# huggingface/distil-whisper

Hardware: AMD Instinct MI355X
Metric: training audio-seconds/s (distil-large-v3 student, 30 s clips) (higher is better)
Workload: dtype bf16

## Files before the change

### distil_whisper_amd/build.py

```python
import os
import subprocess
import sys

HERE = os.path.dirname(os.path.abspath(__file__))
CSRC = os.path.join(HERE, "csrc")
LIB = os.path.join(HERE, "libdwamd.so")
SOURCES = ["gemm.hip", "gemm_tile256.hip", "gemm_tile128.hip", "gemm_wp8_nn.hip", "gemm_wp8_nt.hip", "gemm_wp8_m320.hip", "gemm_wp8_m128.hip",
           "gemm_wp16_nn.hip", "gemm_wp16_tt.hip", "gemm_wp16_small.hip", "gemm_skinny.hip", "attention.hip", "norm.hip", "loss.hip", "logmel.hip", "elementwise.hip", "optim.hip", "decode.hip", "beam.hip", "align.hip", "score.hip", "dropout.hip", "assist.hip"]
FLAGS = ["--offload-arch=gfx950", "-O3", "-std=c++17", "-fPIC", "-ffp-contract=fast", "-munsafe-fp-atomics"]


def kernels_sha16() -> str:
    import hashlib
    h = hashlib.sha256()
    files = sorted(os.path.join(CSRC, f) for f in os.listdir(CSRC) if f.endswith((".hip", ".h")))
    files.append(os.path.join(HERE, "..", "include", "dwamd.h"))
    for f in files:
        h.update(os.path.basename(f).encode())
        with open(f, "rb") as fh:
            h.update(fh.read())
    return h.hexdigest()[:16]


def _stale(obj, deps):
    if not os.path.exists(obj):
        return True
    t = os.path.getmtime(obj)
    return any(os.path.getmtime(d) > t for d in deps)


def build(force: bool = False, verbose: bool = False) -> str:
    hipcc = os.environ.get("HIPCC", "/opt/rocm/bin/hipcc")
    objdir = os.path.join(HERE, "build")
    os.makedirs(objdir, exist_ok=True)
    headers = [os.path.join(CSRC, "common.h"), os.path.join(CSRC, "gemm_common.h"), os.path.join(CSRC, "gemm_kernel.h"), os.path.join(CSRC, "gemm_wp.h"), os.path.join(CSRC, "gemm_wp16.h"), os.path.join(CSRC, "select_rules.h"),
               os.path.join(HERE, "..", "include", "dwamd.h")]
    objs, procs = [], []
    flags = FLAGS + (["-DDW_ABLATE"] if os.environ.get("DW_ABLATE") else [])
    flags += os.environ.get("DW_EXTRA_FLAGS", "").split()
    for src in SOURCES:
        s = os.path.join(CSRC, src)
        o = os.path.join(objdir, src.replace(".hip", ".o"))
        objs.append(o)
        if force or _stale(o, [s] + headers):
            cmd = [hipcc] + flags + ["-c", s, "-o", o]
            if verbose:
                print(" ".join(cmd))
            procs.append((src, subprocess.Popen(cmd, stdout=subprocess.PIPE, stderr=subprocess.STDOUT)))
    for src, p in procs:
        out, _ = p.communicate()
        if p.returncode != 0:
            sys.stderr.write(out.decode())
            raise RuntimeError(f"hipcc failed on {src}")
    if force or procs or _stale(LIB, objs):
        cmd = [hipcc, "--offload-arch=gfx950", "-shared", "-fPIC", "-o", LIB] + objs
        subprocess.check_call(cmd)
    return LIB



if __name__ == "__main__":
    print(build(force="--force" in sys.argv, verbose=True))
```

### distil_whisper_amd/csrc/attention.hip

```cpp
#include "common.h"
#include "../../include/dwamd.h"

#define NEG_BIG (-1.0e30f)
#ifndef DW_ATTN_DEFER
#define DW_ATTN_DEFER 8
#endif
#ifndef DW_ATTN_IDLE_SKIP
#define DW_ATTN_IDLE_SKIP 1
#endif
typedef __attribute__((ext_vector_type(4))) unsigned u32x4;

struct AttnP {
    const bf16* q; const bf16* k; const bf16* v; bf16* o; float* lse;
    const bf16* d_o; float* delta; bf16* dq; bf16* dk; bf16* dv;
    long ldq, ldk, ldv, ldo, lddo, lddq, lddk, lddv;
    int B, H, Lq, Lk;
    long q_rows, kv_rows;
    float* dq_colsum;
    float* dv_colsum;
    const int* q_start; const int* q_len;
    const int* kv_start; const int* kv_len;
    int kv_B;
    int plain_order;
    float defer;
    int coff;
    float scale;
};

__device__ __forceinline__ bf16x8 pack8(const f32x16& x, int s2) {
    bf16x8 r;
#pragma unroll
    for (int e = 0; e < 8; ++e) r[e] = f2bf(x[s2 * 8 + e]);
    return r;
}

__device__ __forceinline__ bf16x8 ldg8(const bf16* base, long row, long ld, int col) {
    return *(const bf16x8*)(base + row * ld + col);
}

__device__ __forceinline__ void store_t(bf16* base, long ld, long row, bool ok, int cb, int hi, const f32x16& a,
                                        float mul) {
    if (!ok) return;
#pragma unroll
    for (int g = 0; g < 4; ++g) {
        bf16x4 w;
#pragma unroll
        for (int e = 0; e < 4; ++e) w[e] = f2bf(a[g * 4 + e] * mul);
#ifdef DW_NT_ATTN
        __builtin_nontemporal_store(w, (bf16x4*)(base + row * ld + cb * 32 + g * 8 + hi * 4));
#else
        *(bf16x4*)(base + row * ld + cb * 32 + g * 8 + hi * 4) = w;
#endif
    }
}

#ifndef DW_ATTN_ROWSTORE
#define DW_ATTN_ROWSTORE 1
#endif
__device__ __forceinline__ void store_rows(bf16* base, long ld, int row0, int nrows, char* patch, int lane,
                                           const f32x16& a0, const f32x16& a1, float mul) {
    const int hi = lane >> 5, ln = lane & 31;
    char* const wr = patch + ln * 144 + hi * 8;
#pragma unroll
    for (int cb = 0; cb < 2; ++cb) {
        const f32x16& a = cb == 0 ? a0 : a1;
#pragma unroll
        for (int g = 0; g < 4; ++g) {
            bf16x4 w;
#pragma unroll
            for (int e = 0; e < 4; ++e) w[e] = f2bf(a[g * 4 + e] * mul);
            *(bf16x4*)(wr + cb * 64 + g * 16) = w;
        }
    }
    const int rr = lane >> 3, sc = lane & 7;
    u32x4 o[4];
#pragma unroll
    for (int it = 0; it < 4; ++it) o[it] = *(const u32x4*)(patch + (it * 8 + rr) * 144 + sc * 16);
    const unsigned loff = (unsigned)(rr * (int)ld + sc * 8) * 2u;
    char* const rb = (char*)(base + (long)row0 * ld);
#pragma unroll
    for (int it = 0; it < 4; ++it)
        if (row0 + it * 8 + rr < nrows) *(u32x4*)(rb + (long)it * 8 * ld * 2 + loff) = o[it];
}

__device__ __forceinline__ void colsum_t(float* colsum, bool ok, int cb, int hi, int ln, const f32x16& a, float mul) {
#pragma unroll
    for (int r = 0; r < 16; ++r) {
        float v = ok ? bf2f(f2bf(a[r] * mul)) : 0.f;
#pragma unroll
        for (int o = 1; o < 32; o <<= 1) v += __shfl_xor(v, o);
        if (ln == 0) atomicAdd(colsum + cb * 32 + (r & 3) + 8 * (r >> 2) + 4 * hi, v);
    }
}

__device__ __forceinline__ void attn_workgroup(int ntile, int H, bool plain, int& tile, int& h, int& b) {
    const int n = gridDim.x, L = blockIdx.x;
    const int xcd = L & 7, slot = L >> 3, q = n >> 3, r = n & 7;
    const int logical = plain ? L : xcd * q + min(xcd, r) + slot;
    tile = logical % ntile;
    const int bh = logical / ntile;
    h = bh % H;
    b = bh / H;
}

template <bool CAUSAL, int NW = 4, int ABL = 0, bool VL = false>
__global__ __launch_bounds__(64 * NW, CAUSAL ? 2 : 4) void attn_fwd_kernel(const AttnP p) {
    __shared__ __attribute__((aligned(1024))) char smem[2 * 16384];
    const int lane = threadIdx.x & 63;
    const int wave = __builtin_amdgcn_readfirstlane(threadIdx.x >> 6);
    const int hi = lane >> 5, ln = lane & 31;
    int tile, h, b;
    attn_workgroup((p.Lq + 32 * NW - 1) / (32 * NW), p.H, p.plain_order, tile, h, b);
    const int qb0 = tile * (32 * NW);
    long q_row0 = (long)b * p.q_rows, kv_row0 = (long)b * p.kv_rows;
    int Lq = p.Lq, Lk = p.Lk;
    if constexpr (VL) {
        q_row0 = p.q_start[b];
        Lq = p.q_len[b];
        if (p.kv_start) { kv_row0 = p.kv_start[b]; Lk = p.kv_len[b]; }
        else kv_row0 = (long)min(b, p.kv_B - 1) * p.kv_rows;
        if (qb0 >= Lq) return;
    }
    const int q = qb0 + wave * 32 + ln;
    const bool q_ok = q < Lq;
    const int qc = q_ok ? q : Lq - 1;
    const bf16* Q = p.q + q_row0 * p.ldq + h * 64;
    const bf16* K = p.k + kv_row0 * p.ldk + h * 64;
    const bf16* V = p.v + kv_row0 * p.ldv + h * 64;

    bf16x8 qf[4];
#pragma unroll
    for (int kk = 0; kk < 4; ++kk) qf[kk] = ldg8(Q, qc, p.ldq, kk * 16 + hi * 8);

    int nkt = (Lk + 63) >> 6;
    if (CAUSAL) {
        const int lim = ((min(qb0 + 32 * NW - 1, Lq - 1) + p.coff) >> 6) + 1;
        nkt = min(nkt, lim);
    }
    const float c = p.scale * 1.4426950408889634f;
    float m_run = NEG_BIG, l_run = 0.f;
    f32x16 o[2];
#pragma unroll
    for (int r = 0; r < 16; ++r) { o[0][r] = 0.f; o[1][r] = 0.f; }

    stage_tile64<NW>(K, p.ldk, 0, Lk, smem, wave, lane);
    stage_tile64<NW>(V, p.ldv, 0, Lk, smem + 8192, wave, lane);
    for (int kt = 0; kt < nkt; ++kt) {
        const int buf = kt & 1;
        if (!(ABL & 16) || kt == 0) {
            wait_vm0_seen();
            __syncthreads();
        }
        if (kt + 1 < nkt && !(ABL & 8)) {
            stage_tile64<NW>(K, p.ldk, (kt + 1) * 64, Lk, smem + (buf ^ 1) * 16384, wave, lane);
            stage_tile64<NW>(V, p.ldv, (kt + 1) * 64, Lk, smem + (buf ^ 1) * 16384 + 8192, wave, lane);
        }
        const char* tK = smem + buf * 16384;
        const char* tV = tK + 8192;
        if (DW_ATTN_IDLE_SKIP && qb0 + wave * 32 >= Lq) continue;
        f32x16 s[2];
#pragma unroll
        for (int kb = 0; kb < 2; ++kb) {
#pragma unroll
            for (int r = 0; r < 16; ++r) s[kb][r] = (ABL & 32) ? o[kb][r] : 0.f;
            if (!(ABL & 32)) {
#pragma unroll
                for (int kk = 0; kk < 4; ++kk)
                    s[kb] = __builtin_amdgcn_mfma_f32_32x32x16_bf16((ABL & 2) ? qf[kk ^ kb] : frag_rows(tK, kb, kk, lane), qf[kk], s[kb], 0, 0, 0);
            }
        }
        const int wq0 = qb0 + wave * 32 + (CAUSAL ? p.coff : 0);
        const bool need_mask = ((kt + 1) * 64 > Lk) || (CAUSAL && kt * 64 + 63 > wq0);
        if (CAUSAL && kt * 64 > wq0 + 31) continue;
        float mx = NEG_BIG;
        if (need_mask) {
#pragma unroll
            for (int kb = 0; kb < 2; ++kb)
#pragma unroll
                for (int r = 0; r < 16; ++r) {
                    const int key = kt * 64 + kb * 32 + (r & 3) + 8 * (r >> 2) + 4 * hi;
                    const bool ok = key < Lk && (!CAUSAL || key <= q + p.coff);
                    s[kb][r] = ok ? s[kb][r] : NEG_BIG;
                }
        }
#pragma unroll
        for (int kb = 0; kb < 2; ++kb)
#pragma unroll
            for (int r = 0; r < 16; ++r) mx = fmaxf(mx, s[kb][r]);
        mx = xhalf_max(mx);
        const bool move = __any((mx - m_run) * c > p.defer);
        const float m_new = move ? fmaxf(m_run, mx) : m_run;
        const float mc = m_new * c;
        f32x2 rs2[2] = {{0.f, 0.f}, {0.f, 0.f}};
        const f32x2 c2 = {c, c}, mc2 = {mc, mc};
#pragma unroll
        for (int kb = 0; kb < 2; ++kb)
#pragma unroll
            for (int r = 0; r < 16; r += 2) {
                f32x2 t = {s[kb][r], s[kb][r + 1]};
                t = t * c2 - mc2;
                f32x2 pv = {__builtin_amdgcn_exp2f(t[0]), __builtin_amdgcn_exp2f(t[1])};
                if (ABL & 1) pv = t;
                s[kb][r] = pv[0];
                s[kb][r + 1] = pv[1];
                rs2[(r >> 1) & 1] += pv;
            }
        rs2[0] += rs2[1];
        float rs = rs2[0][0] + rs2[0][1];
        rs = xhalf_sum(rs);
        if (move) {
            const float alpha = __builtin_amdgcn_exp2f((m_run - m_new) * c);
            l_run *= alpha;
#pragma unroll
            for (int r = 0; r < 16; ++r) { o[0][r] *= alpha; o[1][r] *= alpha; }
        }
        l_run += rs;
        m_run = m_new;
#pragma unroll
        for (int kb = 0; kb < 2; ++kb)
#pragma unroll
            for (int s2 = 0; s2 < 2; ++s2) {
                const bf16x8 pf = pack8(s[kb], s2);
                const int rb = kb * 32 + s2 * 16 + hi * 4;
                if (ABL & 64) {
                    o[kb][s2] += bf2f(pf[0]) + bf2f(pf[2]) + bf2f(pf[4]) + bf2f(pf[6]);
                    continue;
                }
#pragma unroll
                for (int db = 0; db < 2; ++db)
                    o[db] = __builtin_amdgcn_mfma_f32_32x32x16_bf16((ABL & 4) ? qf[db * 2 + s2] : frag_tr(tV, db, rb, rb + 8, lane), pf, o[db], 0, 0, 0);
            }
    }
    const float inv = 1.0f / l_run;
    bf16* O = p.o + q_row0 * p.ldo + h * 64;
    if (DW_ATTN_ROWSTORE && NW <= 7 && (p.ldo & 7) == 0 && ((uintptr_t)p.o & 15) == 0) {
        __syncthreads();
        store_rows(O, p.ldo, qb0 + wave * 32, Lq, smem + wave * 4608, lane, o[0], o[1], inv);
    } else {
        store_t(O, p.ldo, q, q_ok, 0, hi, o[0], inv);
        store_t(O, p.ldo, q, q_ok, 1, hi, o[1], inv);
    }
    if (!VL && p.lse && q_ok && hi == 0) p.lse[((long)b * p.H + h) * Lq + q] = m_run * p.scale + __logf(l_run);
}

template <int NW = 4, int OCC = 3>
__global__ __launch_bounds__(64 * NW, OCC) void attn_fwd_pipe_kernel(const AttnP p) {
    __shared__ __attribute__((aligned(1024))) char smem[3 * 16384];
    const int lane = threadIdx.x & 63;
    const int wave = __builtin_amdgcn_readfirstlane(threadIdx.x >> 6);
    const int hi = lane >> 5, ln = lane & 31;
    int tile, h, b;
    attn_workgroup((p.Lq + 32 * NW - 1) / (32 * NW), p.H, p.plain_order, tile, h, b);
    const int qb0 = tile * (32 * NW);
    const int q = qb0 + wave * 32 + ln;
    const bool q_ok = q < p.Lq;
    const int qc = q_ok ? q : p.Lq - 1;
    const bf16* Q = p.q + (long)b * p.q_rows * p.ldq + h * 64;
    const bf16* K = p.k + (long)b * p.kv_rows * p.ldk + h * 64;
    const bf16* V = p.v + (long)b * p.kv_rows * p.ldv + h * 64;
    bf16x8 qf[4];
#pragma unroll
    for (int kk = 0; kk < 4; ++kk) qf[kk] = ldg8(Q, qc, p.ldq, kk * 16 + hi * 8);
    const int nkt = (p.Lk + 63) >> 6;
    const float c = p.scale * 1.4426950408889634f;
    float m_run = NEG_BIG, l_run = 0.f;
    f32x16 o[2];
#pragma unroll
    for (int r = 0; r < 16; ++r) { o[0][r] = 0.f; o[1][r] = 0.f; }

    auto stage = [&](int kt, int st) __attribute__((always_inline)) {
        stage_tile64<NW>(K, p.ldk, kt * 64, p.Lk, smem + st * 16384, wave, lane);
        stage_tile64<NW>(V, p.ldv, kt * 64, p.Lk, smem + st * 16384 + 8192, wave, lane);
    };
    auto scores = [&](int kt, int st, f32x16 (&s)[2]) __attribute__((always_inline)) {
        const char* tK = smem + st * 16384;
#pragma unroll
        for (int kb = 0; kb < 2; ++kb) {
#pragma unroll
            for (int r = 0; r < 16; ++r) s[kb][r] = 0.f;
#pragma unroll
            for (int kk = 0; kk < 4; ++kk)
                s[kb] = __builtin_amdgcn_mfma_f32_32x32x16_bf16(frag_rows(tK, kb, kk, lane), qf[kk], s[kb], 0, 0, 0);
        }
        if ((kt + 1) * 64 > p.Lk) {
#pragma unroll
            for (int kb = 0; kb < 2; ++kb)
#pragma unroll
                for (int r = 0; r < 16; ++r) {
                    const int key = kt * 64 + kb * 32 + (r & 3) + 8 * (r >> 2) + 4 * hi;
                    s[kb][r] = key < p.Lk ? s[kb][r] : NEG_BIG;
                }
        }
    };
    auto softmax_pv = [&](int st, f32x16 (&s)[2]) __attribute__((always_inline)) {
        const char* tV = smem + st * 16384 + 8192;
        float mx = NEG_BIG;
#pragma unroll
        for (int kb = 0; kb < 2; ++kb)
#pragma unroll
            for (int r = 0; r < 16; ++r) mx = fmaxf(mx, s[kb][r]);
        mx = xhalf_max(mx);
        const bool move = __any((mx - m_run) * c > p.defer);
        const float m_new = move ? fmaxf(m_run, mx) : m_run;
        const float mc = m_new * c;
        f32x2 rs2[2] = {{0.f, 0.f}, {0.f, 0.f}};
        const f32x2 c2 = {c, c}, mc2 = {mc, mc};
#pragma unroll
        for (int kb = 0; kb < 2; ++kb)
#pragma unroll
            for (int r = 0; r < 16; r += 2) {
                f32x2 t = {s[kb][r], s[kb][r + 1]};
                t = t * c2 - mc2;
                const f32x2 pv = {__builtin_amdgcn_exp2f(t[0]), __builtin_amdgcn_exp2f(t[1])};
                s[kb][r] = pv[0];
                s[kb][r + 1] = pv[1];
                rs2[(r >> 1) & 1] += pv;
            }
        rs2[0] += rs2[1];
        float rs = rs2[0][0] + rs2[0][1];
        rs = xhalf_sum(rs);
        if (move) {
            const float alpha = __builtin_amdgcn_exp2f((m_run - m_new) * c);
            l_run *= alpha;
#pragma unroll
            for (int r = 0; r < 16; ++r) { o[0][r] *= alpha; o[1][r] *= alpha; }
        }
        l_run += rs;
        m_run = m_new;
#pragma unroll
        for (int kb = 0; kb < 2; ++kb)
#pragma unroll
            for (int s2 = 0; s2 < 2; ++s2) {
                const bf16x8 pf = pack8(s[kb], s2);
                const int rb = kb * 32 + s2 * 16 + hi * 4;
#pragma unroll
                for (int db = 0; db < 2; ++db)
                    o[db] = __builtin_amdgcn_mfma_f32_32x32x16_bf16(frag_tr(tV, db, rb, rb + 8, lane), pf, o[db], 0, 0, 0);
            }
    };

    stage(0, 0);
    if (nkt > 1) stage(1, 1);
    wait_vm0_seen();
    __syncthreads();
    f32x16 sa[2], sb[2];
    scores(0, 0, sa);
    auto iter = [&](int kt, int st0, int st1, int st2, f32x16 (&cur)[2], f32x16 (&nxt)[2]) __attribute__((always_inline)) {
        if (kt > 0) {
            wait_vm0_seen();
            __syncthreads();
        }
        if (kt + 2 < nkt) stage(kt + 2, st2);
        if (kt + 1 < nkt) scores(kt + 1, st1, nxt);
        softmax_pv(st0, cur);
    };
    int st0 = 0, st1 = 1, st2 = 2;
    for (int kt = 0; kt < nkt; kt += 2) {
        iter(kt, st0, st1, st2, sa, sb);
        if (kt + 1 < nkt) iter(kt + 1, st1, st2, st0, sb, sa);
        const int t0 = st0; st0 = st2; st2 = st1; st1 = t0;
    }
    const float inv = 1.0f / l_run;
    bf16* O = p.o + (long)b * p.q_rows * p.ldo + h * 64;
    if (DW_ATTN_ROWSTORE && (p.ldo & 7) == 0 && ((uintptr_t)p.o & 15) == 0) {
        __syncthreads();
        store_rows(O, p.ldo, qb0 + wave * 32, p.Lq, smem + wave * 4608, lane, o[0], o[1], inv);
    } else {
        store_t(O, p.ldo, q, q_ok, 0, hi, o[0], inv);
        store_t(O, p.ldo, q, q_ok, 1, hi, o[1], inv);
    }
    if (p.lse && q_ok && hi == 0) p.lse[((long)b * p.H + h) * p.Lq + q] = m_run * p.scale + __logf(l_run);
}

template <int NW, bool PRE>
__global__ __launch_bounds__(64 * NW) void attn_decode_kernel(const AttnP p) {
    extern __shared__ __attribute__((aligned(16))) float dsm[];
    const int lane = threadIdx.x & 63;
    const int wave = __builtin_amdgcn_readfirstlane(threadIdx.x >> 6);
    const int h = blockIdx.y, b = blockIdx.z;
    const int sub = lane >> 3, ds = (lane & 7) * 8;
    float* sc = dsm;
    float* part = dsm + ((p.Lk + 3) & ~3);
    float* redm = part + NW * 64;
    float* redl = redm + NW;
    const bf16* Q = p.q + (long)b * p.q_rows * p.ldq + h * 64 + ds;
    const bf16* K = p.k + (long)b * p.kv_rows * p.ldk + h * 64 + ds;
    const bf16* V = p.v + (long)b * p.kv_rows * p.ldv + h * 64 + ds;
    const float c = p.scale * 1.4426950408889634f;
    float qv[8];
    {
        const bf16x8 q8 = *(const bf16x8*)Q;
#pragma unroll
        for (int e = 0; e < 8; ++e) qv[e] = bf2f(q8[e]) * c;
    }
    constexpr int NIT = 12;
    bf16x8 kr[PRE ? NIT : 1], vr[PRE ? NIT : 1];
    if constexpr (PRE) {
#pragma unroll
        for (int it = 0; it < NIT; ++it) {
            int k = wave * 8 + it * (NW * 8) + sub;
            k = k < p.Lk ? k : p.Lk - 1;
            kr[it] = ld_stream<2>((const bf16x8*)(K + (long)k * p.ldk));
        }
#pragma unroll
        for (int it = 0; it < NIT; ++it) {
            int k = wave * 8 + it * (NW * 8) + sub;
            k = k < p.Lk ? k : p.Lk - 1;
            vr[it] = ld_stream<2>((const bf16x8*)(V + (long)k * p.ldv));
        }
    }
    float mx = NEG_BIG;
    float sreg[PRE ? NIT : 1];
    if constexpr (PRE) {
#pragma unroll
        for (int it = 0; it < NIT; ++it) {
            const int k = wave * 8 + it * (NW * 8) + sub;
            float s = 0.f;
#pragma unroll
            for (int e = 0; e < 8; ++e) s = fmaf(qv[e], bf2f(kr[it][e]), s);
            s += __shfl_xor(s, 1);
            s += __shfl_xor(s, 2);
            s += __shfl_xor(s, 4);
            sreg[it] = s;
            if (k < p.Lk) mx = fmaxf(mx, s);
        }
    } else {
    for (int k0 = wave * 8; k0 < p.Lk; k0 += NW * 8) {
        const int k = k0 + sub;
        float s = 0.f;
        if (k < p.Lk) {
            const bf16x8 k8 = *(const bf16x8*)(K + (long)k * p.ldk);
#pragma unroll
            for (int e = 0; e < 8; ++e) s = fmaf(qv[e], bf2f(k8[e]), s);
        }
        s += __shfl_xor(s, 1);
        s += __shfl_xor(s, 2);
        s += __shfl_xor(s, 4);
        if (k < p.Lk) {
            if ((lane & 7) == 0) sc[k] = s;
            mx = fmaxf(mx, s);
        }
    }
    }
    mx = wave_max(mx);
    if (lane == 0) redm[wave] = mx;
    __syncthreads();
    mx = redm[0];
#pragma unroll
    for (int i = 1; i < NW; ++i) mx = fmaxf(mx, redm[i]);
    float o[8] = {0.f, 0.f, 0.f, 0.f, 0.f, 0.f, 0.f, 0.f};
    float l = 0.f;
    if constexpr (PRE) {
#pragma unroll
        for (int it = 0; it < NIT; ++it) {
            const int k = wave * 8 + it * (NW * 8) + sub;
            if (k < p.Lk) {
                const float pv = __builtin_amdgcn_exp2f(sreg[it] - mx);
                l += pv;
                const float pb = round_bf16(pv);
#pragma unroll
                for (int e = 0; e < 8; ++e) o[e] = fmaf(pb, bf2f(vr[it][e]), o[e]);
            }
        }
    } else {
    for (int k0 = wave * 8; k0 < p.Lk; k0 += NW * 8) {
        const int k = k0 + sub;
        if (k < p.Lk) {
            const float pv = __builtin_amdgcn_exp2f(sc[k] - mx);
            l += pv;
            const float pb = round_bf16(pv);
            const bf16x8 v8 = *(const bf16x8*)(V + (long)k * p.ldv);
#pragma unroll
            for (int e = 0; e < 8; ++e) o[e] = fmaf(pb, bf2f(v8[e]), o[e]);
        }
    }
    }
    l = (lane & 7) == 0 ? l : 0.f;
    l = wave_sum(l);
#pragma unroll
    for (int e = 0; e < 8; ++e) {
        o[e] += __shfl_xor(o[e], 8);
        o[e] += __shfl_xor(o[e], 16);
        o[e] += __shfl_xor(o[e], 32);
    }
    if (sub == 0) {
#pragma unroll
        for (int e = 0; e < 8; ++e) part[wave * 64 + ds + e] = o[e];
    }
    if (lane == 0) redl[wave] = l;
    __syncthreads();
    if (wave == 0) {
        float acc = 0.f, lt = 0.f;
#pragma unroll
        for (int i = 0; i < NW; ++i) { acc += part[i * 64 + lane]; lt += redl[i]; }
        bf16* O = p.o + (long)b * p.q_rows * p.ldo + h * 64;
        O[lane] = f2bf(acc / lt);
        if (p.lse && lane == 0) p.lse[(long)b * p.H + h] = (mx + __log2f(lt)) * 0.6931471805599453f;
    }
}

template <bool CAUSAL, bool FS, int NW = 4>
__global__ __launch_bounds__(64 * NW, 3) void attn_bwd_dq_kernel(const AttnP p) {
    __shared__ __attribute__((aligned(1024))) char smem[2 * 16384];
    const int lane = threadIdx.x & 63;
    const int wave = __builtin_amdgcn_readfirstlane(threadIdx.x >> 6);
    const int hi = lane >> 5, ln = lane & 31;
    int tile, h, b;
    attn_workgroup((p.Lq + 32 * NW - 1) / (32 * NW), p.H, p.plain_order, tile, h, b);
    const int qb0 = tile * (32 * NW);
    const int q = qb0 + wave * 32 + ln;
    const bool q_ok = q < p.Lq;
    const int qc = q_ok ? q : p.Lq - 1;
    const bf16* Q = p.q + (long)b * p.Lq * p.ldq + h * 64;
    const bf16* DO = p.d_o + (long)b * p.Lq * p.lddo + h * 64;
    const bf16* K = p.k + (long)b * p.Lk * p.ldk + h * 64;
    const bf16* V = p.v + (long)b * p.Lk * p.ldv + h * 64;

    bf16x8 qf[4], gf[4];
#pragma unroll
    for (int kk = 0; kk < 4; ++kk) {
        qf[kk] = ldg8(Q, qc, p.ldq, kk * 16 + hi * 8);
        gf[kk] = ldg8(DO, qc, p.lddo, kk * 16 + hi * 8);
    }
    const long sidx = ((long)b * p.H + h) * p.Lq + qc;
    const float c = p.scale * 1.4426950408889634f;
    float dsum = 0.f;
    {
        const bf16* Orow = p.o + (long)b * p.Lq * p.ldo + h * 64;
#pragma unroll
        for (int kk = 0; kk < 4; ++kk) {
            const bf16x8 o8 = ldg8(Orow, qc, p.ldo, kk * 16 + hi * 8);
#pragma unroll
            for (int e = 0; e < 8; ++e) dsum += bf2f(o8[e]) * bf2f(gf[kk][e]);
        }
        dsum = xhalf_sum(dsum);
    }
    const float s0 = -p.lse[sidx] / p.scale;
    const float dp0 = -dsum;
    if (q_ok && hi == 0) {
        p.delta[sidx] = dp0;
        p.delta[(long)p.B * p.H * p.Lq + sidx] = s0;
    }

    int nkt = (p.Lk + 63) >> 6;
    if (CAUSAL) nkt = min(nkt, (min(qb0 + 32 * NW - 1, p.Lq - 1) >> 6) + 1);
    f32x16 acc[2];
#pragma unroll
    for (int r = 0; r < 16; ++r) { acc[0][r] = 0.f; acc[1][r] = 0.f; }

    stage_tile64<NW, FS>(K, p.ldk, 0, p.Lk, smem, wave, lane);
    stage_tile64<NW, FS>(V, p.ldv, 0, p.Lk, smem + 8192, wave, lane);
    auto tiles = [&](auto modec, int kt_begin, int kt_end) __attribute__((always_inline)) {
    constexpr int MODE = decltype(modec)::value;
    int lane_o = lane;
    asm volatile("" : "+v"(lane_o));
    const int hi_o = lane_o >> 5, q_o = qb0 + wave * 32 + (lane_o & 31);
    for (int kt = kt_begin; kt < kt_end; ++kt) {
        const int buf = kt & 1;
        wait_vm0();
        __syncthreads();
        if (kt + 1 < nkt) {
            int lane_s = lane_o;
            asm volatile("" : "+v"(lane_s));
            stage_tile64<NW, FS>(K, p.ldk, (kt + 1) * 64, p.Lk, smem + (buf ^ 1) * 16384, wave, lane_s);
            stage_tile64<NW, FS>(V, p.ldv, (kt + 1) * 64, p.Lk, smem + (buf ^ 1) * 16384 + 8192, wave, lane_s);
        }
        const char* tK = smem + buf * 16384;
        const char* tV = tK + 8192;
        const int wq0 = qb0 + wave * 32;
        const bool need_mask = MODE == 1 || (MODE == 2 && (((kt + 1) * 64 > p.Lk) || (CAUSAL && kt * 64 + 63 > wq0)));
        if (CAUSAL && kt * 64 > wq0 + 31) continue;
        if (DW_ATTN_IDLE_SKIP && wq0 >= p.Lq) continue;
#pragma unroll
        for (int kb = 0; kb < 2; ++kb) {
            f32x16 s, dp;
#pragma unroll
            for (int r = 0; r < 16; ++r) { s[r] = s0; dp[r] = dp0; }
#pragma unroll
            for (int kk = 0; kk < 4; ++kk) {
                s = __builtin_amdgcn_mfma_f32_32x32x16_bf16(frag_rows(tK, kb, kk, lane), qf[kk], s, 0, 0, 0);
                dp = __builtin_amdgcn_mfma_f32_32x32x16_bf16(frag_rows(tV, kb, kk, lane), gf[kk], dp, 0, 0, 0);
            }
            const f32x2 c2 = {c, c};
#pragma unroll
            for (int r = 0; r < 16; r += 2) {
                f32x2 t = {s[r], s[r + 1]};
                t = t * c2;
                f32x2 pv = {__builtin_amdgcn_exp2f(t[0]), __builtin_amdgcn_exp2f(t[1])};
                if (need_mask) {
#pragma unroll
                    for (int e = 0; e < 2; ++e) {
                        const int key = kt * 64 + kb * 32 + ((r + e) & 3) + 8 * ((r + e) >> 2) + 4 * hi_o;
                        pv[e] = (key < p.Lk && (!CAUSAL || key <= q_o)) ? pv[e] : 0.f;
                    }
                }
                const f32x2 d2 = {dp[r], dp[r + 1]};
                pv = pv * d2;
                s[r] = pv[0];
                s[r + 1] = pv[1];
            }
#pragma unroll
            for (int s2 = 0; s2 < 2; ++s2) {
                const bf16x8 df = pack8(s, s2);
                const int rb = kb * 32 + s2 * 16 + hi * 4;
#pragma unroll
                for (int db = 0; db < 2; ++db)
                    acc[db] = __builtin_amdgcn_mfma_f32_32x32x16_bf16(frag_tr(tK, db, rb, rb + 8, lane), df, acc[db], 0, 0, 0);
            }
        }
    }
    };
    if constexpr (CAUSAL) tiles(std::integral_constant<int, 2>{}, 0, nkt);
    else {
        const int nfull = p.Lk >> 6;
        tiles(std::integral_constant<int, 0>{}, 0, nfull);
        tiles(std::integral_constant<int, 1>{}, nfull, nkt);
    }
    bf16* DQ = p.dq + (long)b * p.Lq * p.lddq + h * 64;
    if (DW_ATTN_ROWSTORE && NW <= 7 && (p.lddq & 7) == 0 && ((uintptr_t)p.dq & 15) == 0) {
        __syncthreads();
        store_rows(DQ, p.lddq, qb0 + wave * 32, p.Lq, smem + wave * 4608, lane, acc[0], acc[1], p.scale);
    } else {
        store_t(DQ, p.lddq, q, q_ok, 0, hi, acc[0], p.scale);
        store_t(DQ, p.lddq, q, q_ok, 1, hi, acc[1], p.scale);
    }
    if (p.dq_colsum) {
        colsum_t(p.dq_colsum + ((long)b * p.H + h) * 64, q_ok, 0, hi, ln, acc[0], p.scale);
        colsum_t(p.dq_colsum + ((long)b * p.H + h) * 64, q_ok, 1, hi, ln, acc[1], p.scale);
    }
}

template <bool CAUSAL, bool FS, int OCC, int NW = 4>
__global__ __launch_bounds__(64 * NW, OCC) void attn_bwd_dkv_kernel(const AttnP p) {
    constexpr int STG = 16384 + 512;
    __shared__ __attribute__((aligned(1024))) char smem[2 * 17408];
    const int lane = threadIdx.x & 63;
    const int wave = __builtin_amdgcn_readfirstlane(threadIdx.x >> 6);
    const int hi = lane >> 5, ln = lane & 31;
    int tile, h, b;
    attn_workgroup((p.Lk + 32 * NW - 1) / (32 * NW), p.H, p.plain_order, tile, h, b);
    const int kb0 = tile * (32 * NW);
    const int key = kb0 + wave * 32 + ln;
    const bool k_ok = key < p.Lk;
    const int kc = k_ok ? key : p.Lk - 1;
    const bf16* Q = p.q + (long)b * p.Lq * p.ldq + h * 64;
    const bf16* DO = p.d_o + (long)b * p.Lq * p.lddo + h * 64;
    const bf16* K = p.k + (long)b * p.Lk * p.ldk + h * 64;
    const bf16* V = p.v + (long)b * p.Lk * p.ldv + h * 64;
    const float* DEL = p.delta + ((long)b * p.H + h) * p.Lq;
    const float* LSE = DEL + (long)p.B * p.H * p.Lq;

    bf16x8 kf[4], vf[4];
#pragma unroll
    for (int kk = 0; kk < 4; ++kk) {
        kf[kk] = ldg8(K, kc, p.ldk, kk * 16 + hi * 8);
        vf[kk] = ldg8(V, kc, p.ldv, kk * 16 + hi * 8);
    }
    const float c = p.scale * 1.4426950408889634f;
    const int nqt = (p.Lq + 63) >> 6;
    int qt0 = 0;
    if (CAUSAL) qt0 = kb0 >> 6;
    f32x16 av[2], ak[2];
#pragma unroll
    for (int r = 0; r < 16; ++r) { av[0][r] = 0.f; av[1][r] = 0.f; ak[0][r] = 0.f; ak[1][r] = 0.f; }

    auto stage = [&](int qt, int buf, int lane) __attribute__((always_inline)) {
        char* base = smem + buf * 17408;
        stage_tile64<NW, FS>(Q, p.ldq, qt * 64, p.Lq, base, wave, lane);
        stage_tile64<NW, FS>(DO, p.lddo, qt * 64, p.Lq, base + 8192, wave, lane);
        if (wave < 2) {
            int qi = qt * 64 + lane;
            qi = qi < p.Lq ? qi : p.Lq - 1;
            glds4_so(wave == 0 ? LSE : DEL, (unsigned)qi * 4u, lds_addr_of(base + 16384) + (wave == 0 ? 0 : 256));
        }
    };

    if (qt0 < nqt) stage(qt0, 0, lane);
    const int wk0 = kb0 + wave * 32;
    auto tiles = [&](auto modec, int qt_begin, int qt_end) __attribute__((always_inline)) {
    constexpr int MODE = decltype(modec)::value;
    int lane_o = lane;
    asm volatile("" : "+v"(lane_o));
    const int hi_o = lane_o >> 5, key_o = kb0 + wave * 32 + (lane_o & 31);
    const bool k_ok_o = key_o < p.Lk;
    for (int qt = qt_begin; qt < qt_end; ++qt) {
        const int buf = (qt - qt0) & 1;
        wait_vm0_seen();
        __syncthreads();
        if (qt + 1 < nqt) {
            int lane_s = lane_o;
            asm volatile("" : "+v"(lane_s));
            stage(qt + 1, buf ^ 1, lane_s);
        }
        const char* tQ = smem + buf * 17408;
        const char* tG = tQ + 8192;
        const float* tL = (const float*)(tQ + 16384);
        const float* tD = tL + 64;
        const bool need_mask = MODE == 1 || (MODE == 2 && (((qt + 1) * 64 > p.Lq) || (wk0 + 31 >= p.Lk) || (CAUSAL && wk0 + 31 > qt * 64)));
        if (CAUSAL && wk0 > qt * 64 + 63) continue;
        if (DW_ATTN_IDLE_SKIP && wk0 >= p.Lk) continue;
#pragma unroll
        for (int qb = 0; qb < 2; ++qb) {
            f32x16 s, dp;
#pragma unroll
            for (int g = 0; g < 4; ++g) {
                const int ql = qb * 32 + g * 8 + hi * 4;
                const f32x4 l4 = *(const f32x4*)(tL + ql);
                const f32x4 d4 = *(const f32x4*)(tD + ql);
#pragma unroll
                for (int e = 0; e < 4; ++e) { s[g * 4 + e] = l4[e]; dp[g * 4 + e] = d4[e]; }
            }
#pragma unroll
            for (int kk = 0; kk < 4; ++kk) {
                s = __builtin_amdgcn_mfma_f32_32x32x16_bf16(frag_rows(tQ, qb, kk, lane), kf[kk], s, 0, 0, 0);
                dp = __builtin_amdgcn_mfma_f32_32x32x16_bf16(frag_rows(tG, qb, kk, lane), vf[kk], dp, 0, 0, 0);
            }
            f32x16 pr;
            const f32x2 c2 = {c, c};
#pragma unroll
            for (int r = 0; r < 16; r += 2) {
                f32x2 t = {s[r], s[r + 1]};
                t = t * c2;
                f32x2 pv = {__builtin_amdgcn_exp2f(t[0]), __builtin_amdgcn_exp2f(t[1])};
                if (need_mask) {
#pragma unroll
                    for (int e = 0; e < 2; ++e) {
                        const int qi = qt * 64 + qb * 32 + ((r + e) & 3) + 8 * ((r + e) >> 2) + 4 * hi_o;
                        pv[e] = (qi < p.Lq && k_ok_o && (!CAUSAL || key_o <= qi)) ? pv[e] : 0.f;
                    }
                }
                pr[r] = pv[0];
                pr[r + 1] = pv[1];
                const f32x2 d2 = {dp[r], dp[r + 1]};
                pv = pv * d2;
                s[r] = pv[0];
                s[r + 1] = pv[1];
            }
#pragma unroll
            for (int s2 = 0; s2 < 2; ++s2) {
                const bf16x8 pf = pack8(pr, s2);
                const bf16x8 df = pack8(s, s2);
                const int rb = qb * 32 + s2 * 16 + hi * 4;
#pragma unroll
                for (int db = 0; db < 2; ++db) {
                    av[db] = __builtin_amdgcn_mfma_f32_32x32x16_bf16(frag_tr(tG, db, rb, rb + 8, lane), pf, av[db], 0, 0, 0);
                    ak[db] = __builtin_amdgcn_mfma_f32_32x32x16_bf16(frag_tr(tQ, db, rb, rb + 8, lane), df, ak[db], 0, 0, 0);
                }
            }
        }
    }
    };
    if constexpr (CAUSAL) tiles(std::integral_constant<int, 2>{}, qt0, nqt);
    else {
        const int nfull = kb0 + 32 * NW - 1 >= p.Lk ? 0 : (p.Lq >> 6);
        tiles(std::integral_constant<int, 0>{}, 0, nfull);
        tiles(std::integral_constant<int, 1>{}, nfull, nqt);
    }
    bf16* DK = p.dk + (long)b * p.Lk * p.lddk + h * 64;
    bf16* DV = p.dv + (long)b * p.Lk * p.lddv + h * 64;
    if (DW_ATTN_ROWSTORE && NW <= 7 && ((p.lddk | p.lddv) & 7) == 0 && (((uintptr_t)p.dk | (uintptr_t)p.dv) & 15) == 0) {
        __syncthreads();
        store_rows(DK, p.lddk, kb0 + wave * 32, p.Lk, smem + wave * 4608, lane, ak[0], ak[1], p.scale);
        store_rows(DV, p.lddv, kb0 + wave * 32, p.Lk, smem + wave * 4608, lane, av[0], av[1], 1.0f);
    } else {
        store_t(DK, p.lddk, key, k_ok, 0, hi, ak[0], p.scale);
        store_t(DK, p.lddk, key, k_ok, 1, hi, ak[1], p.scale);
        store_t(DV, p.lddv, key, k_ok, 0, hi, av[0], 1.0f);
        store_t(DV, p.lddv, key, k_ok, 1, hi, av[1], 1.0f);
    }
    if (p.dv_colsum) {
        colsum_t(p.dv_colsum + ((long)b * p.H + h) * 64, k_ok, 0, hi, ln, av[0], 1.0f);
        colsum_t(p.dv_colsum + ((long)b * p.H + h) * 64, k_ok, 1, hi, ln, av[1], 1.0f);
    }
}

int g_attn_bwd_stage = 5;
int g_attn_bwd_waves = 4;
int g_attn_fwd_waves = 4;
int g_attn_fwd_pipe = 0;
int g_attn_plain_order = 0;
int g_attn_defer = DW_ATTN_DEFER;
int g_attn_ablate = 0;
int g_attn_decode = 1;
static int check_ld(int64_t ld) { return (ld & 7) ? DW_EINVAL : DW_OK; }

extern "C" int dw_attn_fwd_ex(const void* q, const void* k, const void* v, void* o, float* lse, int B, int H, int Lq,
                              int Lk, int64_t ldq, int64_t ldk, int64_t ldv, int64_t ldo, int64_t q_batch_rows,
                              int64_t kv_batch_rows, int causal, float scale, void* stream);

extern "C" int dw_attn_fwd(const void* q, const void* k, const void* v, void* o, float* lse, int B, int H, int Lq,
                           int Lk, int64_t ldq, int64_t ldk, int64_t ldv, int64_t ldo, int causal, float scale,
                           void* stream) {
    if (!lse) return DW_EINVAL;
    return dw_attn_fwd_ex(q, k, v, o, lse, B, H, Lq, Lk, ldq, ldk, ldv, ldo, Lq, Lk, causal, scale, stream);
}

extern "C" int dw_attn_fwd_ex(const void* q, const void* k, const void* v, void* o, float* lse, int B, int H, int Lq,
                              int Lk, int64_t ldq, int64_t ldk, int64_t ldv, int64_t ldo, int64_t q_batch_rows,
                              int64_t kv_batch_rows, int causal, float scale, void* stream) {
    DW_CLEAR_ERR();
    if (!q || !k || !v || !o || B <= 0 || H <= 0 || Lq <= 0 || Lk <= 0) return DW_EINVAL;
    if (q_batch_rows < Lq || kv_batch_rows < Lk) return DW_EINVAL;
    if ((int64_t)Lk * ldk >= (1LL << 31) || (int64_t)Lk * ldv >= (1LL << 31)) return DW_EINVAL;
    if (check_ld(ldq) || check_ld(ldk) || check_ld(ldv) || (ldo & 3)) return DW_EINVAL;
    if (((uintptr_t)q & 15) || ((uintptr_t)k & 15) || ((uintptr_t)v & 15) || ((uintptr_t)o & 7)) return DW_EINVAL;
    AttnP p = {};
    p.q = (const bf16*)q; p.k = (const bf16*)k; p.v = (const bf16*)v; p.o = (bf16*)o; p.lse = lse;
    p.ldq = ldq; p.ldk = ldk; p.ldv = ldv; p.ldo = ldo;
    p.B = B; p.H = H; p.Lq = Lq; p.Lk = Lk; p.scale = scale;
    p.q_rows = q_batch_rows; p.kv_rows = kv_batch_rows;
    if (causal != 0 && causal != 1 && causal != 2) return DW_EINVAL;
    if (causal == 2 && Lk < Lq) return DW_EINVAL;
    p.coff = causal == 2 ? Lk - Lq : 0;
    hipStream_t s = (hipStream_t)stream;
    if (Lq == 1 && causal != 1 && g_attn_decode && Lk <= 8192) {
        const size_t smem = (((size_t)Lk + 3) & ~(size_t)3) * 4 + 16 * 64 * 4 + 2 * 16 * 4;
        if (Lk >= 512 && Lk <= 16 * 8 * 12 && (g_attn_decode & 2))
            hipLaunchKernelGGL((attn_decode_kernel<16, true>), dim3(1, H, B), dim3(1024), smem, s, p);
        else if (Lk >= 512) hipLaunchKernelGGL((attn_decode_kernel<16, false>), dim3(1, H, B), dim3(1024), smem, s, p);
        else hipLaunchKernelGGL((attn_decode_kernel<4, false>), dim3(1, H, B), dim3(256), smem, s, p);
        DW_CHECK_LAUNCH();
        return DW_OK;
    }
    const int g4 = (Lq + 127) / 128;
    dim3 grid(g4 * H * B), block(256);
    p.plain_order = g_attn_plain_order;
    p.defer = (float)g_attn_defer;
#ifdef DW_ABLATE
    if (!causal && g_attn_ablate) {
        switch (g_attn_ablate) {
#define ABLC(v) case v: hipLaunchKernelGGL((attn_fwd_kernel<false, 4, v>), grid, block, 0, s, p); break;
            ABLC(1) ABLC(2) ABLC(4) ABLC(6) ABLC(8) ABLC(24) ABLC(32) ABLC(64) ABLC(7) ABLC(31) ABLC(30)
#undef ABLC
            default: return DW_EINVAL;
        }
        return DW_OK;
    }
#endif
    const int g8 = (Lq + 255) / 256;
    if (causal) hipLaunchKernelGGL(attn_fwd_kernel<true>, grid, block, 0, s, p);
    else if (g_attn_fwd_pipe == 2 && Lk > 64) hipLaunchKernelGGL((attn_fwd_pipe_kernel<4, 2>), grid, block, 0, s, p);
    else if (g_attn_fwd_pipe && Lk > 64) hipLaunchKernelGGL((attn_fwd_pipe_kernel<4, 3>), grid, block, 0, s, p);
    else if (g_attn_fwd_waves == 8 && g8 * 2 == g4 && (long)g8 * H * B >= 512)
        hipLaunchKernelGGL((attn_fwd_kernel<false, 8>), dim3(g8 * H * B), dim3(512), 0, s, p);
    else hipLaunchKernelGGL(attn_fwd_kernel<false>, grid, block, 0, s, p);
    DW_CHECK_LAUNCH();
    return DW_OK;
}

extern "C" int dw_attn_fwd_varlen(const void* q, const void* k, const void* v, void* o, int n_seq, int H, int max_q, int Lk,
                                  int64_t ldq, int64_t ldk, int64_t ldv, int64_t ldo, const int32_t* q_start, const int32_t* q_len,
                                  const int32_t* kv_start, const int32_t* kv_len, int kv_batches, int64_t kv_batch_rows, int causal,
                                  float scale, void* stream) {
    DW_CLEAR_ERR();
    if (!q || !k || !v || !o || !q_start || !q_len || n_seq <= 0 || H <= 0 || max_q <= 0) return DW_EINVAL;
    if ((kv_start == nullptr) != (kv_len == nullptr)) return DW_EINVAL;
    if (!kv_start && (Lk <= 0 || kv_batches <= 0 || kv_batch_rows < Lk || causal)) return DW_EINVAL;
    if (causal != 0 && causal != 1) return DW_EINVAL;
    if (check_ld(ldq) || check_ld(ldk) || check_ld(ldv) || (ldo & 7)) return DW_EINVAL;
    if (((uintptr_t)q & 15) || ((uintptr_t)k & 15) || ((uintptr_t)v & 15) || ((uintptr_t)o & 15)) return DW_EINVAL;
    const int64_t lk_max = kv_start ? max_q : Lk;
    if (lk_max * ldk >= (1LL << 31) || lk_max * ldv >= (1LL << 31)) return DW_EINVAL;
    AttnP p = {};
    p.q = (const bf16*)q; p.k = (const bf16*)k; p.v = (const bf16*)v; p.o = (bf16*)o; p.lse = nullptr;
    p.ldq = ldq; p.ldk = ldk; p.ldv = ldv; p.ldo = ldo;
    p.B = n_seq; p.H = H; p.Lq = max_q; p.Lk = kv_start ? max_q : Lk; p.scale = scale;
    p.q_rows = 0; p.kv_rows = kv_batch_rows; p.coff = 0;
    p.q_start = q_start; p.q_len = q_len; p.kv_start = kv_start; p.kv_len = kv_len; p.kv_B = kv_batches;
    p.plain_order = g_attn_plain_order;
    p.defer = (float)g_attn_defer;
    hipStream_t s = (hipStream_t)stream;
    dim3 grid(((max_q + 127) / 128) * H * n_seq), block(256);
    if (causal) hipLaunchKernelGGL((attn_fwd_kernel<true, 4, 0, true>), grid, block, 0, s, p);
    else hipLaunchKernelGGL((attn_fwd_kernel<false, 4, 0, true>), grid, block, 0, s, p);
    DW_CHECK_LAUNCH();
    return DW_OK;
}

extern "C" int dw_attn_bwd_ex(const void* q, const void* k, const void* v, const void* o, const void* d_o,
                              const float* lse, float* delta, void* dq, void* dk, void* dv, int B, int H, int Lq, int Lk,
                              int64_t ldq, int64_t ldk, int64_t ldv, int64_t ldo, int64_t lddo, int64_t lddq,
                              int64_t lddk, int64_t lddv, int causal, float scale, float* dq_colsum, float* dv_colsum,
                              void* stream);
extern "C" int dw_attn_bwd(const void* q, const void* k, const void* v, const void* o, const void* d_o,
                           const float* lse, float* delta, void* dq, void* dk, void* dv, int B, int H, int Lq, int Lk,
                           int64_t ldq, int64_t ldk, int64_t ldv, int64_t ldo, int64_t lddo, int64_t lddq,
                           int64_t lddk, int64_t lddv, int causal, float scale, void* stream) {
    return dw_attn_bwd_ex(q, k, v, o, d_o, lse, delta, dq, dk, dv, B, H, Lq, Lk, ldq, ldk, ldv, ldo, lddo, lddq, lddk, lddv,
                          causal, scale, nullptr, nullptr, stream);
}

extern "C" int dw_attn_bwd_ex(const void* q, const void* k, const void* v, const void* o, const void* d_o,
                              const float* lse, float* delta, void* dq, void* dk, void* dv, int B, int H, int Lq, int Lk,
                              int64_t ldq, int64_t ldk, int64_t ldv, int64_t ldo, int64_t lddo, int64_t lddq,
                              int64_t lddk, int64_t lddv, int causal, float scale, float* dq_colsum, float* dv_colsum,
                              void* stream) {
    DW_CLEAR_ERR();
    if (!q || !k || !v || !o || !d_o || !lse || !delta || !dq || !dk || !dv) return DW_EINVAL;
    if (B <= 0 || H <= 0 || Lq <= 0 || Lk <= 0) return DW_EINVAL;
    if (causal != 0 && causal != 1) return DW_EINVAL;
    if (check_ld(ldq) || check_ld(ldk) || check_ld(ldv) || check_ld(ldo) || check_ld(lddo)) return DW_EINVAL;
    if ((lddq & 3) || (lddk & 3) || (lddv & 3)) return DW_EINVAL;
    if ((int64_t)Lk * ldk >= (1LL << 31) || (int64_t)Lk * ldv >= (1LL << 31) || (int64_t)Lq * ldq >= (1LL << 31) ||
        (int64_t)Lq * lddo >= (1LL << 31))
        return DW_EINVAL;
    if (((uintptr_t)q & 15) || ((uintptr_t)k & 15) || ((uintptr_t)v & 15) || ((uintptr_t)o & 15) ||
        ((uintptr_t)d_o & 15) || ((uintptr_t)dq & 7) || ((uintptr_t)dk & 7) || ((uintptr_t)dv & 7))
        return DW_EINVAL;
    AttnP p = {};
    p.q = (const bf16*)q; p.k = (const bf16*)k; p.v = (const bf16*)v; p.o = (bf16*)o; p.lse = (float*)lse;
    p.d_o = (const bf16*)d_o; p.delta = delta; p.dq = (bf16*)dq; p.dk = (bf16*)dk; p.dv = (bf16*)dv;
    p.ldq = ldq; p.ldk = ldk; p.ldv = ldv; p.ldo = ldo; p.lddo = lddo; p.lddq = lddq; p.lddk = lddk; p.lddv = lddv;
    p.B = B; p.H = H; p.Lq = Lq; p.Lk = Lk; p.scale = scale;
    p.dq_colsum = dq_colsum; p.dv_colsum = dv_colsum;
    hipStream_t s = (hipStream_t)stream;
    const int q4 = (Lq + 127) / 128, k4 = (Lk + 127) / 128;
    dim3 gq(q4 * H * B), gk(k4 * H * B), block(256);
    p.plain_order = g_attn_plain_order;
    p.defer = (float)g_attn_defer;
    const int fs = g_attn_bwd_stage;
    if (causal) {
        hipLaunchKernelGGL((attn_bwd_dq_kernel<true, false>), gq, block, 0, s, p);
        hipLaunchKernelGGL((attn_bwd_dkv_kernel<true, false, 2>), gk, block, 0, s, p);
    } else {
        const int q12 = (Lq + 383) / 384, k12 = (Lk + 383) / 384;
        const bool dq12 = g_attn_bwd_waves == 12 && q12 * 3 == q4 && (long)q12 * H * B >= 256;
        const bool dkv12 = g_attn_bwd_waves == 12 && k12 * 3 == k4 && (long)k12 * H * B >= 256;
        if (dq12) hipLaunchKernelGGL((attn_bwd_dq_kernel<false, true, 12>), dim3(q12 * H * B), dim3(768), 0, s, p);
        else if (fs & 1) hipLaunchKernelGGL((attn_bwd_dq_kernel<false, true>), gq, block, 0, s, p);
        else hipLaunchKernelGGL((attn_bwd_dq_kernel<false, false>), gq, block, 0, s, p);
        if (dkv12) hipLaunchKernelGGL((attn_bwd_dkv_kernel<false, false, 3, 12>), dim3(k12 * H * B), dim3(768), 0, s, p);
        else if ((fs & 6) == 6) hipLaunchKernelGGL((attn_bwd_dkv_kernel<false, true, 3>), gk, block, 0, s, p);
        else if (fs & 4) hipLaunchKernelGGL((attn_bwd_dkv_kernel<false, false, 3>), gk, block, 0, s, p);
        else if (fs & 2) hipLaunchKernelGGL((attn_bwd_dkv_kernel<false, true, 2>), gk, block, 0, s, p);
        else hipLaunchKernelGGL((attn_bwd_dkv_kernel<false, false, 2>), gk, block, 0, s, p);
    }
    DW_CHECK_LAUNCH();
    return DW_OK;
}
```

### distil_whisper_amd/csrc/common.h

```cpp
#pragma once
#include <hip/hip_runtime.h>
#include <stdint.h>
#include <type_traits>

typedef __bf16 bf16;
typedef __attribute__((ext_vector_type(8))) __bf16 bf16x8;
typedef __attribute__((ext_vector_type(4))) __bf16 bf16x4;
typedef __attribute__((ext_vector_type(4))) _Float16 f16x4;
typedef __attribute__((ext_vector_type(2))) __bf16 bf16x2;
typedef __attribute__((ext_vector_type(16))) float f32x16;
typedef __attribute__((ext_vector_type(4))) float f32x4;
typedef __attribute__((address_space(3))) void lds_void_t;
typedef __attribute__((address_space(1))) void glb_void_t;
typedef __attribute__((address_space(3))) bf16x4 lds_bf16x4_t;

#define DW_WAVE 64

template <int B, int E, class F>
__device__ __forceinline__ void static_for(F&& f) {
    if constexpr (B < E) {
        f(std::integral_constant<int, B>{});
        static_for<B + 1, E>(f);
    }
}

__device__ __forceinline__ float bf2f(bf16 x) { return (float)x; }
__device__ __forceinline__ bf16 f2bf(float x) { return (bf16)x; }
__device__ __forceinline__ float round_bf16(float x) { return (float)((bf16)x); }
__device__ __forceinline__ float bits2f(unsigned short u) {
    return __uint_as_float(((unsigned)u) << 16);
}

__device__ __forceinline__ float gelu_f(float x) { return 0.5f * x * (1.0f + erff(x * 0.70710678118654752f)); }
__device__ __forceinline__ float gelu_grad_f(float x) {
    const float cdf = 0.5f * (1.0f + erff(x * 0.70710678118654752f));
    const float pdf = 0.39894228040143268f * __expf(-0.5f * x * x);
    return cdf + x * pdf;
}

typedef __attribute__((ext_vector_type(2))) float f32x2;
__device__ __forceinline__ void gelu_parts2(f32x2 x, f32x2& cdf, f32x2& pdf) {
    f32x2 ax; ax[0] = fabsf(x[0]); ax[1] = fabsf(x[1]);
    const f32x2 u = ax * 0.70710678118654752f;
    f32x2 den = u * 0.3275911f + 1.0f;
    f32x2 t; t[0] = __builtin_amdgcn_rcpf(den[0]); t[1] = __builtin_amdgcn_rcpf(den[1]);
    const f32x2 xx = x * x * -0.72134752044448170f;
    f32x2 e; e[0] = __builtin_amdgcn_exp2f(xx[0]); e[1] = __builtin_amdgcn_exp2f(xx[1]);
    f32x2 y = t * 1.061405429f + (-1.453152027f);
    y = y * t + 1.421413741f;
    y = y * t + (-0.284496736f);
    y = y * t + 0.254829592f;
    const f32x2 tail = y * t * e;
    f32x2 half_tail = tail * 0.5f;
    cdf[0] = x[0] >= 0.f ? 1.0f - half_tail[0] : half_tail[0];
    cdf[1] = x[1] >= 0.f ? 1.0f - half_tail[1] : half_tail[1];
    pdf = e * 0.39894228040143268f;
}
__device__ __forceinline__ void gelu_y_s_pdf2(f32x2 x, f32x2& y, f32x2& s, f32x2& pdf) {
    f32x2 ax; ax[0] = fabsf(x[0]); ax[1] = fabsf(x[1]);
    const f32x2 u = ax * 0.70710678118654752f;
    f32x2 den = u * 0.3275911f + 1.0f;
    f32x2 t; t[0] = __builtin_amdgcn_rcpf(den[0]); t[1] = __builtin_amdgcn_rcpf(den[1]);
    const f32x2 xx = x * x * -0.72134752044448170f;
    f32x2 e; e[0] = __builtin_amdgcn_exp2f(xx[0]); e[1] = __builtin_amdgcn_exp2f(xx[1]);
    f32x2 yy = t * 1.061405429f + (-1.453152027f);
    yy = yy * t + 1.421413741f;
    yy = yy * t + (-0.284496736f);
    yy = yy * t + 0.254829592f;
    const f32x2 tail = yy * t * e;
    s = 1.0f - tail;
    y = (ax * s + x) * 0.5f;
    pdf = e * 0.39894228040143268f;
}
__device__ __forceinline__ f32x2 gelu_cdf_from_s2(f32x2 x, f32x2 s) {
    f32x2 c;
    c[0] = __builtin_copysignf(s[0], x[0]); c[1] = __builtin_copysignf(s[1], x[1]);
    return c * 0.5f + 0.5f;
}
__device__ __forceinline__ f32x2 round_bf16_pair(f32x2 v) {
    const bf16x2 r = __builtin_convertvector(v, bf16x2);
    const unsigned u = __builtin_bit_cast(unsigned, r);
    f32x2 o; o[0] = __uint_as_float(u << 16); o[1] = __uint_as_float(u & 0xffff0000u);
    return o;
}
__device__ __forceinline__ f32x2 gelu_fast2(f32x2 x) {
    f32x2 y, s, pdf;
    gelu_y_s_pdf2(x, y, s, pdf);
    return y;
}
__device__ __forceinline__ f32x2 gelu_grad_fast2(f32x2 x) {
    f32x2 y, s, pdf;
    gelu_y_s_pdf2(x, y, s, pdf);
    return gelu_cdf_from_s2(x, s) + x * pdf;
}
__device__ __forceinline__ float gelu_fast(float x) { f32x2 v; v[0] = x; v[1] = x; return gelu_fast2(v)[0]; }
__device__ __forceinline__ float gelu_grad_fast(float x) { f32x2 v; v[0] = x; v[1] = x; return gelu_grad_fast2(v)[0]; }

__device__ __forceinline__ int swz7(int row) {
    return (((row >> 1) & 1) << 2) | (((row >> 3) & 1) << 1) | ((row >> 2) & 1);
}

__device__ __forceinline__ void glds16(const void* gsrc, void* lds_wave_base) {
    const unsigned m0v = __builtin_amdgcn_readfirstlane((unsigned)(unsigned long long)(lds_void_t*)lds_wave_base);
    asm volatile("s_mov_b32 m0, %0\n\ts_nop 0\n\tglobal_load_lds_dwordx4 %1, off" :: "s"(m0v), "v"(gsrc) : "memory");
}
__device__ __forceinline__ void glds4(const void* gsrc, void* lds_wave_base) {
    const unsigned m0v = __builtin_amdgcn_readfirstlane((unsigned)(unsigned long long)(lds_void_t*)lds_wave_base);
    asm volatile("s_mov_b32 m0, %0\n\ts_nop 0\n\tglobal_load_lds_dword %1, off" :: "s"(m0v), "v"(gsrc) : "memory");
}

__device__ __forceinline__ void wait_vm0() { asm volatile("s_waitcnt vmcnt(0)" ::: "memory"); }
__device__ __forceinline__ void wait_vm0_seen() {
    __builtin_amdgcn_s_waitcnt(0x0F70);
    asm volatile("" ::: "memory");
}
__device__ __forceinline__ float xhalf_max(float v) {
    const auto r = __builtin_amdgcn_permlane32_swap(__float_as_uint(v), __float_as_uint(v), false, false);
    return fmaxf(__uint_as_float(r[0]), __uint_as_float(r[1]));
}
__device__ __forceinline__ float xhalf_sum(float v) {
    const auto r = __builtin_amdgcn_permlane32_swap(__float_as_uint(v), __float_as_uint(v), false, false);
    return __uint_as_float(r[0]) + __uint_as_float(r[1]);
}

__device__ __forceinline__ bf16x8 frag_rows(const char* tile, int rb, int kk, int lane) {
    const int row = rb * 32 + (lane & 31);
    const int ps = ((kk << 1) | (lane >> 5)) ^ swz7(row);
    return *(const bf16x8*)(tile + row * 128 + ps * 16);
}

__device__ __forceinline__ bf16x8 frag_tr(const char* tile, int cb, int rowbase0, int rowbase1, int lane) {
    const int g = lane >> 4, p = lane & 15;
    const int col = cb * 32 + ((g & 1) << 4) + ((p & 3) << 2);
    const int r0 = rowbase0 + (p >> 2);
    const int r1 = rowbase1 + (p >> 2);
    const int ls = col >> 3;
    const int inb = (p & 1) << 3;
    const char* a0 = tile + r0 * 128 + ((ls ^ swz7(r0)) << 4) + inb;
    const char* a1 = tile + r1 * 128 + ((ls ^ swz7(r1)) << 4) + inb;
    bf16x4 lo = __builtin_amdgcn_ds_read_tr16_b64_v4bf16((lds_bf16x4_t*)a0);
    bf16x4 hi = __builtin_amdgcn_ds_read_tr16_b64_v4bf16((lds_bf16x4_t*)a1);
    bf16x8 r;
    r[0] = lo[0]; r[1] = lo[1]; r[2] = lo[2]; r[3] = lo[3];
    r[4] = hi[0]; r[5] = hi[1]; r[6] = hi[2]; r[7] = hi[3];
    return r;
}

__device__ __forceinline__ void glds16_so(const void* sbase, unsigned voff, unsigned lds_addr) {
    asm volatile("s_mov_b32 m0, %0\n\ts_nop 0\n\tglobal_load_lds_dwordx4 %1, %2" :: "s"(lds_addr), "v"(voff), "s"(sbase) : "memory");
}
__device__ __forceinline__ void glds4_so(const void* sbase, unsigned voff, unsigned lds_addr) {
    asm volatile("s_mov_b32 m0, %0\n\ts_nop 0\n\tglobal_load_lds_dword %1, %2" :: "s"(lds_addr), "v"(voff), "s"(sbase) : "memory");
}
__device__ __forceinline__ unsigned lds_addr_of(const void* lds) {
    return __builtin_amdgcn_readfirstlane((unsigned)(unsigned long long)(lds_void_t*)lds);
}
template <int NW, bool FAST = true>
__device__ __forceinline__ void stage_tile64(const bf16* base, long row_stride, int row0, int nrows, char* lds,
                                             int wave, int lane) {
    static_assert(NW == 4 || NW == 8 || NW == 12 || NW == 2, "chunk c = wave + i * NW: rows 8 c + (lane >> 3)");
    const int ld = (int)row_stride;
    const unsigned lds0 = __builtin_amdgcn_readfirstlane((unsigned)(unsigned long long)(lds_void_t*)lds);
    if (row0 + 64 <= nrows) {
        const int row = wave * 8 + (lane >> 3);
        const unsigned voff = (unsigned)(row * ld + (((lane & 7) ^ swz7(row)) << 3)) * 2u;
#pragma unroll
        for (int c = wave; c < 8; c += NW) {
            const bf16* tb = base + (long)__builtin_amdgcn_readfirstlane((row0 + (c - wave) * 8) * ld);
            glds16_so(tb, voff, lds0 + c * 1024);
        }
    } else {
#pragma unroll
        for (int c = wave; c < 8; c += NW) {
            const int row = c * 8 + (lane >> 3);
            const int ls = (lane & 7) ^ swz7(row);
            int grow = row0 + row;
            grow = grow < nrows ? grow : nrows - 1;
            glds16_so(base, (unsigned)(grow * ld + ls * 8) * 2u, lds0 + c * 1024);
        }
    }
}

__device__ __forceinline__ float wave_sum(float v) {
#pragma unroll
    for (int o = 32; o > 0; o >>= 1) v += __shfl_xor(v, o);
    return v;
}
__device__ __forceinline__ float wave_max(float v) {
#pragma unroll
    for (int o = 32; o > 0; o >>= 1) v = fmaxf(v, __shfl_xor(v, o));
    return v;
}

template <int NT>
__device__ __forceinline__ float block_sum(float v, float* red) {
    v = wave_sum(v);
    const int wave = threadIdx.x >> 6, lane = threadIdx.x & 63;
    __syncthreads();
    if (lane == 0) red[wave] = v;
    __syncthreads();
    float t = 0.f;
#pragma unroll
    for (int i = 0; i < NT / 64; ++i) t += red[i];
    return t;
}
template <int NT>
__device__ __forceinline__ float block_max(float v, float* red) {
    v = wave_max(v);
    const int wave = threadIdx.x >> 6, lane = threadIdx.x & 63;
    __syncthreads();
    if (lane == 0) red[wave] = v;
    __syncthreads();
    float t = red[0];
#pragma unroll
    for (int i = 1; i < NT / 64; ++i) t = fmaxf(t, red[i]);
    return t;
}

#define DW_CLEAR_ERR() (void)hipGetLastError()
#define DW_CHECK_LAUNCH()                                  \
    do {                                                   \
        hipError_t e__ = hipGetLastError();                \
        if (e__ != hipSuccess) return (int)e__;            \
    } while (0)

#ifndef DW_DECODE_NT
#define DW_DECODE_NT 2
#endif
template <int BIT, class T>
__device__ __forceinline__ T ld_stream(const T* p) {
    if constexpr ((DW_DECODE_NT & BIT) != 0) return __builtin_nontemporal_load(p);
    else return *p;
}
```

### distil_whisper_amd/csrc/gemm.hip

```cpp
#include "gemm_common.h"
#include <mutex>
#include <unordered_map>

bool dw_gemm_skinny_ok(const GemmP& p, int trans_a, int trans_b);
int dw_gemm_skinny_launch(const GemmP& p, hipStream_t s);
int dw_gemm_tile256_launch(const GemmP& p, int ta, int tb, hipStream_t s);
int dw_gemm_tile128_launch(const GemmP& p, int ta, int tb, hipStream_t s);
int dw_gemm_wp8_nn_launch(const GemmP& p, hipStream_t s);
int dw_gemm_wp8_nt_launch(const GemmP& p, hipStream_t s);
int dw_gemm_wp8_nn320_launch(const GemmP& p, hipStream_t s);
int dw_gemm_wp8_nt320_launch(const GemmP& p, hipStream_t s);
int dw_gemm_wp8_nn128_launch(const GemmP& p, hipStream_t s);
int dw_gemm_wp8_nt128_launch(const GemmP& p, hipStream_t s);
int dw_gemm_wp16_nn_launch(const GemmP& p, hipStream_t s);
int dw_gemm_wp16_tt_launch(const GemmP& p, hipStream_t s);
int dw_gemm_wp16_nn_small_launch(const GemmP& p, hipStream_t s);
int dw_gemm_wp16_nt_small_launch(const GemmP& p, hipStream_t s);

extern int g_attn_bwd_stage;
extern int g_attn_decode;
extern int g_attn_ablate;
extern int g_attn_fwd_waves;
extern int g_attn_fwd_pipe;
extern int g_attn_plain_order;
extern int g_attn_defer;
extern int g_attn_bwd_waves;
extern int g_logmel_mfma;
extern int g_decode_fuse_off;
extern int g_skinny_wide;
extern int g_ln_variant;
enum { GEMM_RULE = 0,
       GEMM_REFERENCE = 1,
       GEMM_FORCE_320 = 2 };
static int g_gemm_mode = GEMM_RULE;
int g_gemm_strip = 0;
int g_gemm_cus = 256;
static int g_gemm_stage_next = 1;
static int g_gemm_dynamic = 1;
static int g_gemm_small_m = 1;
static int g_gemm_row_tail = 1;

static int* gemm_sched_slot(hipStream_t s) {
    static std::mutex mu;
    static std::unordered_map<hipStream_t, int*> slots;
    std::lock_guard<std::mutex> lock(mu);
    auto it = slots.find(s);
    if (it != slots.end()) return it->second;
    hipStreamCaptureStatus st = hipStreamCaptureStatusNone;
    if (hipStreamIsCapturing(s, &st) != hipSuccess || st != hipStreamCaptureStatusNone) { (void)hipGetLastError(); return nullptr; }
    int* ptr = nullptr;
    if (hipMalloc((void**)&ptr, 64) != hipSuccess || hipMemsetAsync(ptr, 0, 64, s) != hipSuccess) { (void)hipGetLastError(); return nullptr; }
    slots[s] = ptr;
    return ptr;
}
int g_gemm_strip_budget = 4;
extern "C" int dw_debug_set(int key, int value) {
    if (key == 0) { if (value < GEMM_RULE || value > GEMM_FORCE_320) return DW_EINVAL; g_gemm_mode = value; return DW_OK; }
    if (key == 1) { g_gemm_strip = value; return DW_OK; }
    if (key == 3) { g_attn_bwd_stage = value; return DW_OK; }
    if (key == 4) { g_attn_decode = value; return DW_OK; }
    if (key == 5) { g_logmel_mfma = value; return DW_OK; }
    if (key == 6) { g_gemm_strip_budget = value; return DW_OK; }
    if (key == 7) { g_decode_fuse_off = value; return DW_OK; }
    if (key == 8) { g_skinny_wide = value; return DW_OK; }
    if (key == 10) { g_gemm_dynamic = value; return DW_OK; }
    if (key == 11) { g_gemm_stage_next = value; return DW_OK; }
    if (key == 17) { g_attn_bwd_waves = value; return DW_OK; }
    if (key == 21) { g_ln_variant = value; return DW_OK; }
    if (key == 22) { g_gemm_row_tail = value; return DW_OK; }
    if (key == 25) { if (value < 0 || value > 1) return DW_EINVAL; g_gemm_small_m = value; return DW_OK; }
    if (key == 26) { g_attn_fwd_pipe = value; return DW_OK; }
    if (key == 18) { g_attn_plain_order = value; return DW_OK; }
    if (key == 23) { if (value < 0 || value > 64) return DW_EINVAL; g_attn_defer = value; return DW_OK; }
    if (key == 16) { g_attn_fwd_waves = value; return DW_OK; }
    if (key == 15) { g_attn_ablate = value; return DW_OK; }
    if (key == 9) { if (value < 8 || value > 256 || (value & 7)) return DW_EINVAL; g_gemm_cus = value; return DW_OK; }
    return DW_EINVAL;
}

__global__ __launch_bounds__(256) void reduce_slices_kernel(const float* part, long stride, int slices, float* out,
                                                            long n, int accumulate) {
    const long i = ((long)blockIdx.x * 256 + threadIdx.x) * 4;
    if (i >= n) return;
    f32x4 acc = accumulate ? *(const f32x4*)(out + i) : f32x4{0.f, 0.f, 0.f, 0.f};
    for (int s = 0; s < slices; ++s) {
        const f32x4 v = *(const f32x4*)(part + s * stride + i);
#pragma unroll
        for (int e = 0; e < 4; ++e) acc[e] += v[e];
    }
    *(f32x4*)(out + i) = acc;
}

extern "C" int dw_reduce_slices(const float* part, int64_t stride, int slices, float* out, int64_t n, int accumulate,
                                void* stream) {
    DW_CLEAR_ERR();
    if (!part || !out || slices < 1 || n <= 0 || (n & 3) || (stride & 3) || ((uintptr_t)part & 15) ||
        ((uintptr_t)out & 15))
        return DW_EINVAL;
    hipLaunchKernelGGL(reduce_slices_kernel, dim3((n / 4 + 255) / 256), dim3(256), 0, (hipStream_t)stream, part,
                       (long)stride, slices, out, (long)n, accumulate);
    DW_CHECK_LAUNCH();
    return DW_OK;
}

__global__ __launch_bounds__(256) void reduce_slices_ld_kernel(const float* part, long slice_stride, long ld_part, int slices,
                                                               float* out, long ld_out, int rows, int cols4, int accumulate) {
    const long i = (long)blockIdx.x * 256 + threadIdx.x;
    if (i >= (long)rows * cols4) return;
    const int r = (int)(i / cols4), c = (int)(i - (long)r * cols4) * 4;
    float* o = out + (long)r * ld_out + c;
    f32x4 acc = accumulate ? *(const f32x4*)o : f32x4{0.f, 0.f, 0.f, 0.f};
    const float* src = part + (long)r * ld_part + c;
    for (int s = 0; s < slices; ++s) {
        const f32x4 v = *(const f32x4*)(src + s * slice_stride);
#pragma unroll
        for (int e = 0; e < 4; ++e) acc[e] += v[e];
    }
    *(f32x4*)o = acc;
}
extern "C" int dw_reduce_slices_ld(const float* part, int64_t slice_stride, int64_t ld_part, int slices, float* out, int64_t ld_out,
                                   int rows, int cols, int accumulate, void* stream) {
    DW_CLEAR_ERR();
    if (!part || !out || slices < 1 || rows <= 0 || cols <= 0 || (cols & 3) || (ld_part & 3) || (ld_out & 3) || (slice_stride & 3) ||
        ld_part < cols || ld_out < cols || ((uintptr_t)part & 15) || ((uintptr_t)out & 15))
        return DW_EINVAL;
    const long n = (long)rows * (cols / 4);
    hipLaunchKernelGGL(reduce_slices_ld_kernel, dim3((n + 255) / 256), dim3(256), 0, (hipStream_t)stream, part, (long)slice_stride,
                       (long)ld_part, slices, out, (long)ld_out, rows, cols / 4, accumulate);
    DW_CHECK_LAUNCH();
    return DW_OK;
}

enum GemmKernel {
    K_SKINNY,
    K_TILE128,
    K_TILE256,
    K_WP8_M128,
    K_WP16_SMALL,
    K_WP8_320,
    K_WP16_NN,
    K_WP8_NN,
    K_WP8_NT,
    K_WP16_TT,
};

static GemmKernel gemm_choose(const DwGemm* g, const GemmP& p) {
    const bool ta = g->trans_a, tb = g->trans_b, nn = !ta && !tb;
    const bool one_slice = p.split_k == 1 && !p.atomic;
    const bool ref = g_gemm_mode == GEMM_REFERENCE;
    const bool res_f32 = g->r && g->r_dtype == DW_F32 && g->c_dtype == DW_F32;
    const long cus = g_gemm_cus, tn = (g->n + 255) / 256;
    const long t256 = (long)((g->m + 255) / 256) * tn;
    const bool fits320 = !ta && one_slice && g->m % 320 == 0 && g->n % 256 == 0;
    int tile = g->tile;
    if ((tile == 0 || tile == 16) && dw_gemm_skinny_ok(p, ta, tb)) return K_SKINNY;
    bool one_round_320 = false, small_m_256 = false;
    if (tile != 128 && tile != 256) {
        tile = t256 >= 512 ? 256 : 128;
        if (tile == 128 && !ref && g_gemm_small_m && !ta && one_slice) {
            const long r128 = (((long)(g->m + 127) / 128) * tn + cus - 1) / cus;
            const long r256 = (t256 + cus - 1) / cus;
            const long r320 = fits320 ? ((long)(g->m / 320) * tn + cus - 1) / cus : 0;
            const long c128 = r128 * 100, c256 = r256 * 165, c320 = fits320 ? r320 * 205 : (1L << 40);
            if (c320 <= c128 && c320 <= c256) { tile = 256; one_round_320 = true; }
            else if (c256 <= c128) { tile = 256; small_m_256 = true; }
            else return K_WP8_M128;
        }
    }
    if (tile == 256 && g->tile != 256 && nn && res_f32 && g->k <= 1024 && one_slice) tile = 128;
    if (tile == 128) return K_TILE128;
    const long spanA = ta ? (long)g->k * g->lda * 2 : 256L * g->lda * 2 + (long)g->k * 2;
    const long spanB = tb ? (long)g->k * g->ldb * 2 : 256L * g->ldb * 2 + (long)g->k * 2;
    if (ref || spanA >= 0x7fffffffL || spanB >= 0x7fffffffL) return K_TILE256;
    if (small_m_256) return K_WP16_SMALL;
    if (fits320 && (one_round_320 || g_gemm_mode == GEMM_FORCE_320)) return K_WP8_320;
    if (nn && g->k <= 2560 && g->n >= 3840 && !g->r && !g->z_out && !g->zgrad_in && g->c_dtype != DW_F32) return K_WP16_NN;
    if (fits320) {
        const long r256 = (((g->m + 255) / 256) * tn + cus - 1) / cus * 4;
        const long r320 = ((g->m / 320) * tn + cus - 1) / cus * 5;
        if (tb ? r320 < r256 && !g->zgrad_in : r320 <= r256) return K_WP8_320;
    }
    if (nn) return res_f32 && g->k <= 2560 ? K_TILE256 : K_WP8_NN;
    if (!ta) return K_WP8_NT;
    if (tb) return K_WP16_TT;
    return K_TILE256;
}

extern "C" int dw_gemm_bf16(const DwGemm* g, void* stream) {
    DW_CLEAR_ERR();
    if (!g || (!g->a && !g->ln_x) || !g->b || !g->c) return DW_EINVAL;
    if (g->m <= 0 || g->n <= 0 || g->k <= 0 || (g->k & 63)) return DW_EINVAL;
    if ((g->lda & 7) || (g->ldb & 7)) return DW_EINVAL;
    if ((g->a && ((uintptr_t)g->a & 15)) || ((uintptr_t)g->b & 15)) return DW_EINVAL;
    if (g->trans_a && g->lda < ((g->m + 7) & ~7)) return DW_EINVAL;
    if (g->trans_b && g->ldb < ((g->n + 7) & ~7)) return DW_EINVAL;
    GemmP p;
    p.a = (const bf16*)g->a; p.b = (const bf16*)g->b; p.c = g->c; p.bias = g->bias;
    p.z_out = (bf16*)g->z_out; p.zgrad = (const bf16*)g->zgrad_in; p.r = g->r;
    p.lda = g->lda; p.ldb = g->ldb; p.ldc = g->ldc; p.ldz = g->ldz; p.ldzg = g->ldzg; p.ldr = g->ldr;
    p.m = g->m; p.n = g->n; p.k = g->k;
    p.act = g->act; p.c_dtype = g->c_dtype; p.r_dtype = g->r_dtype; p.r_row_mod = g->r_row_mod;
    p.round_res = g->round_res; p.tiles_n = 0; p.nwg = 0;
    p.split_k = g->split_k > 1 ? g->split_k : 1;
    p.atomic = g->atomic_acc ? 1 : 0;
    if (p.split_k > (g->k >> 6)) p.split_k = g->k >> 6;
    p.slice_stride = 0;
    p.sched = nullptr;
    p.zg_f16 = g->z_is_gelu_grad ? 1 : 0;
    p.colsum = g->colsum_out;
    if (g->colsum_out && (g->split_k > 1 || g->atomic_acc || ((uintptr_t)g->colsum_out & 3))) return DW_EINVAL;
    p.stage_next = g_gemm_stage_next;
    if (p.zg_f16 && g->z_out && g->act != 1) return DW_EINVAL;
    p.ln_x = g->ln_x; p.ln_g = g->ln_gamma; p.ln_b = g->ln_beta; p.ld_lnx = g->ld_lnx; p.ln_x_dtype = g->ln_x_dtype;
    p.ln_eps = g->ln_eps;
    p.kv_out = (bf16*)g->kv_out; p.kv_ld = g->kv_ld; p.kv_split = g->kv_split; p.kv_rpb = g->kv_rows_per_batch;
    p.kv_pitch = g->kv_batch_pitch; p.kv_row0 = g->kv_row0;
    const bool fused = g->ln_x || g->kv_out;
    if (g->ln_x && (!g->ln_gamma || !g->ln_beta || g->k > 1280 || g->m > 32 || (g->ld_lnx & 7) ||
                    ((uintptr_t)g->ln_x & 15) || ((uintptr_t)g->ln_gamma & 15) || ((uintptr_t)g->ln_beta & 15)))
        return DW_EINVAL;
    if (g->kv_out && (g->c_dtype != DW_BF16 || g->act || g->r || g->z_out || g->zgrad_in || (g->kv_split & 15) ||
                      g->kv_split <= 0 || g->kv_split >= g->n || g->kv_rows_per_batch <= 0 || (g->kv_ld & 3) ||
                      ((uintptr_t)g->kv_out & 7)))
        return DW_EINVAL;
    if (p.split_k > 1 && !p.atomic) {
        if (g->c_dtype != DW_F32 || g->bias || g->z_out || g->zgrad_in || g->r || g->act || g->slice_stride <= 0)
            return DW_EINVAL;
        p.slice_stride = g->slice_stride;
    }
    if (p.atomic && (g->c_dtype != DW_F32 || g->bias || g->z_out || g->zgrad_in || g->r || g->act)) return DW_EINVAL;
    {
        const int es = g->c_dtype == DW_F32 ? 4 : 2;
        bool v = ((uintptr_t)g->c % (4 * es)) == 0 && (g->ldc & 3) == 0;
        if (g->bias) v = v && ((uintptr_t)g->bias & 15) == 0;
        if (g->z_out) v = v && ((uintptr_t)g->z_out & 7) == 0 && (g->ldz & 3) == 0;
        if (g->zgrad_in) v = v && ((uintptr_t)g->zgrad_in & 7) == 0 && (g->ldzg & 3) == 0;
        if (g->r) v = v && ((uintptr_t)g->r % (g->r_dtype == DW_F32 ? 16 : 8)) == 0 && (g->ldr & 3) == 0;
        p.vec = v ? 1 : 0;
    }
    hipStream_t s = (hipStream_t)stream;
    if (g->tile == 16 && !dw_gemm_skinny_ok(p, g->trans_a, g->trans_b)) return DW_EINVAL;
    const GemmKernel kern = gemm_choose(g, p);
    if (kern == K_SKINNY) {
        if (g->colsum_out) return DW_EINVAL;
        return dw_gemm_skinny_launch(p, s);
    }
    if (fused) return DW_EINVAL;
    if (g->tile == 129 && (g->trans_a || p.split_k != 1 || p.atomic)) return DW_EINVAL;
    if (kern == K_TILE128) return dw_gemm_tile128_launch(p, g->trans_a, g->trans_b, s);
    p.strip = g_gemm_strip;
    if (g_gemm_dynamic) p.sched = gemm_sched_slot(s);
    if (kern == K_WP8_M128) return g->trans_b ? dw_gemm_wp8_nt128_launch(p, s) : dw_gemm_wp8_nn128_launch(p, s);
    if (g->k <= 1024) p.stage_next |= 128;
    switch (kern) {
    case K_WP16_SMALL: return g->trans_b ? dw_gemm_wp16_nt_small_launch(p, s) : dw_gemm_wp16_nn_small_launch(p, s);
    case K_WP8_320: return g->trans_b ? dw_gemm_wp8_nt320_launch(p, s) : dw_gemm_wp8_nn320_launch(p, s);
    case K_WP8_NN: return dw_gemm_wp8_nn_launch(p, s);
    case K_WP8_NT: return dw_gemm_wp8_nt_launch(p, s);
    case K_WP16_TT: return dw_gemm_wp16_tt_launch(p, s);
    case K_WP16_NN: {
        const int tm_full = p.m / 256, rem = p.m - tm_full * 256;
        const long tn = (p.n + 255) / 256;
        const long rounds_all = ((long)(tm_full + 1) * tn + g_gemm_cus - 1) / g_gemm_cus;
        const long rounds_full = ((long)tm_full * tn + g_gemm_cus - 1) / g_gemm_cus;
        if (g_gemm_row_tail && g->tile != 256 && rem > 0 && rem <= 128 && tm_full > 0 && rounds_full < rounds_all && !p.colsum) {
            GemmP q1 = p, q2 = p;
            q1.m = tm_full * 256;
            const size_t es = p.c_dtype == DW_F32 ? 4 : 2;
            q2.m = rem;
            q2.a = p.a + (long)q1.m * p.lda;
            q2.c = (char*)p.c + (size_t)q1.m * p.ldc * es;
            q2.sched = nullptr;
            const int rc1 = dw_gemm_wp16_nn_launch(q1, s);
            if (rc1 != DW_OK) return rc1;
            return dw_gemm_tile128_launch(q2, 0, 0, s);
        }
        return dw_gemm_wp16_nn_launch(p, s);
    }
    default: return dw_gemm_tile256_launch(p, g->trans_a, g->trans_b, s);
    }
}
```

Measured before the change: 2787.

## Split attention tile loops into steady-state and tail paths with precomputed staging offsets

Attention forward, dQ and dKV kernels now run their full, unmasked tiles through a steady-state loop. That loop stages K/V (or Q/dO) with precomputed per-lane LDS and global offsets and drops the bounds checks. The last tile or tiles go through a generic tail loop, which can skip the second 32-key half when it lies entirely past Lk or above the causal limit. The aim is to cut address arithmetic and masking work in the inner loop and to avoid MFMA work on dead halves. The cost is more code duplication and larger kernel code, which could affect register allocation.

```diff
diff --git a/distil_whisper_amd/build.py b/distil_whisper_amd/build.py
--- a/distil_whisper_amd/build.py
+++ b/distil_whisper_amd/build.py
@@ -34,6 +34,7 @@
     objdir = os.path.join(HERE, "build")
     os.makedirs(objdir, exist_ok=True)
     headers = [os.path.join(CSRC, "common.h"), os.path.join(CSRC, "gemm_common.h"), os.path.join(CSRC, "gemm_kernel.h"), os.path.join(CSRC, "gemm_wp.h"), os.path.join(CSRC, "gemm_wp16.h"), os.path.join(CSRC, "select_rules.h"),
+               os.path.join(CSRC, "attention_fwd_tiles.h"), os.path.join(CSRC, "attention_dq_tiles.h"), os.path.join(CSRC, "attention_dkv_tiles.h"),
                os.path.join(HERE, "..", "include", "dwamd.h")]
     objs, procs = [], []
     flags = FLAGS + (["-DDW_ABLATE"] if os.environ.get("DW_ABLATE") else [])
diff --git a/distil_whisper_amd/csrc/attention.hip b/distil_whisper_amd/csrc/attention.hip
--- a/distil_whisper_amd/csrc/attention.hip
+++ b/distil_whisper_amd/csrc/attention.hip
@@ -4,6 +4,9 @@
 #define NEG_BIG (-1.0e30f)
 #ifndef DW_ATTN_DEFER
 #define DW_ATTN_DEFER 8
+#endif
+#ifndef DW_ATTN_HALF_SKIP
+#define DW_ATTN_HALF_SKIP 1
 #endif
 #ifndef DW_ATTN_IDLE_SKIP
 #define DW_ATTN_IDLE_SKIP 1
@@ -23,6 +26,7 @@
     int kv_B;
     int plain_order;
     float defer;
+    int half_skip;
     int coff;
     float scale;
 };
@@ -103,7 +107,7 @@
     b = bh / H;
 }
 
-template <bool CAUSAL, int NW = 4, int ABL = 0, bool VL = false>
+template <bool CAUSAL, int NW = 4, int ABL = 0, bool VL = false, bool GS = false>
 __global__ __launch_bounds__(64 * NW, CAUSAL ? 2 : 4) void attn_fwd_kernel(const AttnP p) {
     __shared__ __attribute__((aligned(1024))) char smem[2 * 16384];
     const int lane = threadIdx.x & 63;
@@ -145,92 +149,24 @@
 
     stage_tile64<NW>(K, p.ldk, 0, Lk, smem, wave, lane);
     stage_tile64<NW>(V, p.ldv, 0, Lk, smem + 8192, wave, lane);
-    for (int kt = 0; kt < nkt; ++kt) {
-        const int buf = kt & 1;
-        if (!(ABL & 16) || kt == 0) {
-            wait_vm0_seen();
-            __syncthreads();
-        }
-        if (kt + 1 < nkt && !(ABL & 8)) {
-            stage_tile64<NW>(K, p.ldk, (kt + 1) * 64, Lk, smem + (buf ^ 1) * 16384, wave, lane);
-            stage_tile64<NW>(V, p.ldv, (kt + 1) * 64, Lk, smem + (buf ^ 1) * 16384 + 8192, wave, lane);
-        }
-        const char* tK = smem + buf * 16384;
-        const char* tV = tK + 8192;
-        if (DW_ATTN_IDLE_SKIP && qb0 + wave * 32 >= Lq) continue;
-        f32x16 s[2];
-#pragma unroll
-        for (int kb = 0; kb < 2; ++kb) {
-#pragma unroll
-            for (int r = 0; r < 16; ++r) s[kb][r] = (ABL & 32) ? o[kb][r] : 0.f;
-            if (!(ABL & 32)) {
-#pragma unroll
-                for (int kk = 0; kk < 4; ++kk)
-                    s[kb] = __builtin_amdgcn_mfma_f32_32x32x16_bf16((ABL & 2) ? qf[kk ^ kb] : frag_rows(tK, kb, kk, lane), qf[kk], s[kb], 0, 0, 0);
-            }
-        }
-        const int wq0 = qb0 + wave * 32 + (CAUSAL ? p.coff : 0);
-        const bool need_mask = ((kt + 1) * 64 > Lk) || (CAUSAL && kt * 64 + 63 > wq0);
-        if (CAUSAL && kt * 64 > wq0 + 31) continue;
-        float mx = NEG_BIG;
-        if (need_mask) {
-#pragma unroll
-            for (int kb = 0; kb < 2; ++kb)
-#pragma unroll
-                for (int r = 0; r < 16; ++r) {
-                    const int key = kt * 64 + kb * 32 + (r & 3) + 8 * (r >> 2) + 4 * hi;
-                    const bool ok = key < Lk && (!CAUSAL || key <= q + p.coff);
-                    s[kb][r] = ok ? s[kb][r] : NEG_BIG;
-                }
-        }
-#pragma unroll
-        for (int kb = 0; kb < 2; ++kb)
-#pragma unroll
-            for (int r = 0; r < 16; ++r) mx = fmaxf(mx, s[kb][r]);
-        mx = xhalf_max(mx);
-        const bool move = __any((mx - m_run) * c > p.defer);
-        const float m_new = move ? fmaxf(m_run, mx) : m_run;
-        const float mc = m_new * c;
-        f32x2 rs2[2] = {{0.f, 0.f}, {0.f, 0.f}};
-        const f32x2 c2 = {c, c}, mc2 = {mc, mc};
-#pragma unroll
-        for (int kb = 0; kb < 2; ++kb)
-#pragma unroll
-            for (int r = 0; r < 16; r += 2) {
-                f32x2 t = {s[kb][r], s[kb][r + 1]};
-                t = t * c2 - mc2;
-                f32x2 pv = {__builtin_amdgcn_exp2f(t[0]), __builtin_amdgcn_exp2f(t[1])};
-                if (ABL & 1) pv = t;
-                s[kb][r] = pv[0];
-                s[kb][r + 1] = pv[1];
-                rs2[(r >> 1) & 1] += pv;
-            }
-        rs2[0] += rs2[1];
-        float rs = rs2[0][0] + rs2[0][1];
-        rs = xhalf_sum(rs);
-        if (move) {
-            const float alpha = __builtin_amdgcn_exp2f((m_run - m_new) * c);
-            l_run *= alpha;
-#pragma unroll
-            for (int r = 0; r < 16; ++r) { o[0][r] *= alpha; o[1][r] *= alpha; }
-        }
-        l_run += rs;
-        m_run = m_new;
-#pragma unroll
-        for (int kb = 0; kb < 2; ++kb)
-#pragma unroll
-            for (int s2 = 0; s2 < 2; ++s2) {
-                const bf16x8 pf = pack8(s[kb], s2);
-                const int rb = kb * 32 + s2 * 16 + hi * 4;
-                if (ABL & 64) {
-                    o[kb][s2] += bf2f(pf[0]) + bf2f(pf[2]) + bf2f(pf[4]) + bf2f(pf[6]);
-                    continue;
-                }
-#pragma unroll
-                for (int db = 0; db < 2; ++db)
-                    o[db] = __builtin_amdgcn_mfma_f32_32x32x16_bf16((ABL & 4) ? qf[db * 2 + s2] : frag_tr(tV, db, rb, rb + 8, lane), pf, o[db], 0, 0, 0);
-            }
-    }
+    const unsigned lds0 = lds_addr_of(smem);
+    const int ks = (GS || CAUSAL) ? 0 : max(min(nkt, Lk >> 6) - 1, 0);
+    if constexpr (!GS && !CAUSAL) {
+#define ATTN_STEADY true
+#define ATTN_KT_BEGIN 0
+#define ATTN_KT_END ks
+#include "attention_fwd_tiles.h"
+#undef ATTN_STEADY
+#undef ATTN_KT_BEGIN
+#undef ATTN_KT_END
+    }
+#define ATTN_STEADY false
+#define ATTN_KT_BEGIN ks
+#define ATTN_KT_END nkt
+#include "attention_fwd_tiles.h"
+#undef ATTN_STEADY
+#undef ATTN_KT_BEGIN
+#undef ATTN_KT_END
     const float inv = 1.0f / l_run;
     bf16* O = p.o + q_row0 * p.ldo + h * 64;
     if (DW_ATTN_ROWSTORE && NW <= 7 && (p.ldo & 7) == 0 && ((uintptr_t)p.o & 15) == 0) {
@@ -499,7 +435,7 @@
     }
 }
 
-template <bool CAUSAL, bool FS, int NW = 4>
+template <bool CAUSAL, bool GS, int NW = 4>
 __global__ __launch_bounds__(64 * NW, 3) void attn_bwd_dq_kernel(const AttnP p) {
     __shared__ __attribute__((aligned(1024))) char smem[2 * 16384];
     const int lane = threadIdx.x & 63;
@@ -548,73 +484,52 @@
 #pragma unroll
     for (int r = 0; r < 16; ++r) { acc[0][r] = 0.f; acc[1][r] = 0.f; }
 
-    stage_tile64<NW, FS>(K, p.ldk, 0, p.Lk, smem, wave, lane);
-    stage_tile64<NW, FS>(V, p.ldv, 0, p.Lk, smem + 8192, wave, lane);
-    auto tiles = [&](auto modec, int kt_begin, int kt_end) __attribute__((always_inline)) {
-    constexpr int MODE = decltype(modec)::value;
-    int lane_o = lane;
-    asm volatile("" : "+v"(lane_o));
-    const int hi_o = lane_o >> 5, q_o = qb0 + wave * 32 + (lane_o & 31);
-    for (int kt = kt_begin; kt < kt_end; ++kt) {
-        const int buf = kt & 1;
-        wait_vm0();
-        __syncthreads();
-        if (kt + 1 < nkt) {
-            int lane_s = lane_o;
-            asm volatile("" : "+v"(lane_s));
-            stage_tile64<NW, FS>(K, p.ldk, (kt + 1) * 64, p.Lk, smem + (buf ^ 1) * 16384, wave, lane_s);
-            stage_tile64<NW, FS>(V, p.ldv, (kt + 1) * 64, p.Lk, smem + (buf ^ 1) * 16384 + 8192, wave, lane_s);
-        }
-        const char* tK = smem + buf * 16384;
-        const char* tV = tK + 8192;
-        const int wq0 = qb0 + wave * 32;
-        const bool need_mask = MODE == 1 || (MODE == 2 && (((kt + 1) * 64 > p.Lk) || (CAUSAL && kt * 64 + 63 > wq0)));
-        if (CAUSAL && kt * 64 > wq0 + 31) continue;
-        if (DW_ATTN_IDLE_SKIP && wq0 >= p.Lq) continue;
-#pragma unroll
-        for (int kb = 0; kb < 2; ++kb) {
-            f32x16 s, dp;
-#pragma unroll
-            for (int r = 0; r < 16; ++r) { s[r] = s0; dp[r] = dp0; }
-#pragma unroll
-            for (int kk = 0; kk < 4; ++kk) {
-                s = __builtin_amdgcn_mfma_f32_32x32x16_bf16(frag_rows(tK, kb, kk, lane), qf[kk], s, 0, 0, 0);
-                dp = __builtin_amdgcn_mfma_f32_32x32x16_bf16(frag_rows(tV, kb, kk, lane), gf[kk], dp, 0, 0, 0);
-            }
-            const f32x2 c2 = {c, c};
-#pragma unroll
-            for (int r = 0; r < 16; r += 2) {
-                f32x2 t = {s[r], s[r + 1]};
-                t = t * c2;
-                f32x2 pv = {__builtin_amdgcn_exp2f(t[0]), __builtin_amdgcn_exp2f(t[1])};
-                if (need_mask) {
-#pragma unroll
-                    for (int e = 0; e < 2; ++e) {
-                        const int key = kt * 64 + kb * 32 + ((r + e) & 3) + 8 * ((r + e) >> 2) + 4 * hi_o;
-                        pv[e] = (key < p.Lk && (!CAUSAL || key <= q_o)) ? pv[e] : 0.f;
-                    }
-                }
-                const f32x2 d2 = {dp[r], dp[r + 1]};
-                pv = pv * d2;
-                s[r] = pv[0];
-                s[r + 1] = pv[1];
-            }
-#pragma unroll
-            for (int s2 = 0; s2 < 2; ++s2) {
-                const bf16x8 df = pack8(s, s2);
-                const int rb = kb * 32 + s2 * 16 + hi * 4;
-#pragma unroll
-                for (int db = 0; db < 2; ++db)
-                    acc[db] = __builtin_amdgcn_mfma_f32_32x32x16_bf16(frag_tr(tK, db, rb, rb + 8, lane), df, acc[db], 0, 0, 0);
-            }
-        }
-    }
-    };
-    if constexpr (CAUSAL) tiles(std::integral_constant<int, 2>{}, 0, nkt);
-    else {
+    stage_tile64<NW>(K, p.ldk, 0, p.Lk, smem, wave, lane);
+    stage_tile64<NW>(V, p.ldv, 0, p.Lk, smem + 8192, wave, lane);
+    const unsigned lds0 = lds_addr_of(smem);
+    if constexpr (CAUSAL) {
+#define ATTN_MODE 2
+#define ATTN_STEADY false
+#define ATTN_KT_BEGIN 0
+#define ATTN_KT_END nkt
+#include "attention_dq_tiles.h"
+#undef ATTN_MODE
+#undef ATTN_STEADY
+#undef ATTN_KT_BEGIN
+#undef ATTN_KT_END
+    } else {
         const int nfull = p.Lk >> 6;
-        tiles(std::integral_constant<int, 0>{}, 0, nfull);
-        tiles(std::integral_constant<int, 1>{}, nfull, nkt);
+        const int ks = GS ? nfull : max(nfull - 1, 0);
+        if constexpr (GS) {
+#define ATTN_MODE 0
+#define ATTN_STEADY false
+#define ATTN_KT_BEGIN 0
+#define ATTN_KT_END nfull
+#include "attention_dq_tiles.h"
+#undef ATTN_MODE
+#undef ATTN_STEADY
+#undef ATTN_KT_BEGIN
+#undef ATTN_KT_END
+        } else {
+#define ATTN_MODE 0
+#define ATTN_STEADY true
+#define ATTN_KT_BEGIN 0
+#define ATTN_KT_END ks
+#include "attention_dq_tiles.h"
+#undef ATTN_MODE
+#undef ATTN_STEADY
+#undef ATTN_KT_BEGIN
+#undef ATTN_KT_END
+        }
+#define ATTN_MODE 1
+#define ATTN_STEADY false
+#define ATTN_KT_BEGIN ks
+#define ATTN_KT_END nkt
+#include "attention_dq_tiles.h"
+#undef ATTN_MODE
+#undef ATTN_STEADY
+#undef ATTN_KT_BEGIN
+#undef ATTN_KT_END
     }
     bf16* DQ = p.dq + (long)b * p.Lq * p.lddq + h * 64;
     if (DW_ATTN_ROWSTORE && NW <= 7 && (p.lddq & 7) == 0 && ((uintptr_t)p.dq & 15) == 0) {
@@ -630,7 +545,7 @@
     }
 }
 
-template <bool CAUSAL, bool FS, int OCC, int NW = 4>
+template <bool CAUSAL, bool GS, int OCC, int NW = 4>
 __global__ __launch_bounds__(64 * NW, OCC) void attn_bwd_dkv_kernel(const AttnP p) {
     constexpr int STG = 16384 + 512;
     __shared__ __attribute__((aligned(1024))) char smem[2 * 17408];
@@ -666,8 +581,8 @@
 
     auto stage = [&](int qt, int buf, int lane) __attribute__((always_inline)) {
         char* base = smem + buf * 17408;
-        stage_tile64<NW, FS>(Q, p.ldq, qt * 64, p.Lq, base, wave, lane);
-        stage_tile64<NW, FS>(DO, p.lddo, qt * 64, p.Lq, base + 8192, wave, lane);
+        stage_tile64<NW>(Q, p.ldq, qt * 64, p.Lq, base, wave, lane);
+        stage_tile64<NW>(DO, p.lddo, qt * 64, p.Lq, base + 8192, wave, lane);
         if (wave < 2) {
             int qi = qt * 64 + lane;
             qi = qi < p.Lq ? qi : p.Lq - 1;
@@ -677,84 +592,50 @@
 
     if (qt0 < nqt) stage(qt0, 0, lane);
     const int wk0 = kb0 + wave * 32;
-    auto tiles = [&](auto modec, int qt_begin, int qt_end) __attribute__((always_inline)) {
-    constexpr int MODE = decltype(modec)::value;
-    int lane_o = lane;
-    asm volatile("" : "+v"(lane_o));
-    const int hi_o = lane_o >> 5, key_o = kb0 + wave * 32 + (lane_o & 31);
-    const bool k_ok_o = key_o < p.Lk;
-    for (int qt = qt_begin; qt < qt_end; ++qt) {
-        const int buf = (qt - qt0) & 1;
-        wait_vm0_seen();
-        __syncthreads();
-        if (qt + 1 < nqt) {
-            int lane_s = lane_o;
-            asm volatile("" : "+v"(lane_s));
-            stage(qt + 1, buf ^ 1, lane_s);
-        }
-        const char* tQ = smem + buf * 17408;
-        const char* tG = tQ + 8192;
-        const float* tL = (const float*)(tQ + 16384);
-        const float* tD = tL + 64;
-        const bool need_mask = MODE == 1 || (MODE == 2 && (((qt + 1) * 64 > p.Lq) || (wk0 + 31 >= p.Lk) || (CAUSAL && wk0 + 31 > qt * 64)));
-        if (CAUSAL && wk0 > qt * 64 + 63) continue;
-        if (DW_ATTN_IDLE_SKIP && wk0 >= p.Lk) continue;
-#pragma unroll
-        for (int qb = 0; qb < 2; ++qb) {
-            f32x16 s, dp;
-#pragma unroll
-            for (int g = 0; g < 4; ++g) {
-                const int ql = qb * 32 + g * 8 + hi * 4;
-                const f32x4 l4 = *(const f32x4*)(tL + ql);
-                const f32x4 d4 = *(const f32x4*)(tD + ql);
-#pragma unroll
-                for (int e = 0; e < 4; ++e) { s[g * 4 + e] = l4[e]; dp[g * 4 + e] = d4[e]; }
-            }
-#pragma unroll
-            for (int kk = 0; kk < 4; ++kk) {
-                s = __builtin_amdgcn_mfma_f32_32x32x16_bf16(frag_rows(tQ, qb, kk, lane), kf[kk], s, 0, 0, 0);
-                dp = __builtin_amdgcn_mfma_f32_32x32x16_bf16(frag_rows(tG, qb, kk, lane), vf[kk], dp, 0, 0, 0);
-            }
-            f32x16 pr;
-            const f32x2 c2 = {c, c};
-#pragma unroll
-            for (int r = 0; r < 16; r += 2) {
-                f32x2 t = {s[r], s[r + 1]};
-                t = t * c2;
-                f32x2 pv = {__builtin_amdgcn_exp2f(t[0]), __builtin_amdgcn_exp2f(t[1])};
-                if (need_mask) {
-#pragma unroll
-                    for (int e = 0; e < 2; ++e) {
-                        const int qi = qt * 64 + qb * 32 + ((r + e) & 3) + 8 * ((r + e) >> 2) + 4 * hi_o;
-                        pv[e] = (qi < p.Lq && k_ok_o && (!CAUSAL || key_o <= qi)) ? pv[e] : 0.f;
-                    }
-                }
-                pr[r] = pv[0];
-                pr[r + 1] = pv[1];
-                const f32x2 d2 = {dp[r], dp[r + 1]};
-                pv = pv * d2;
-                s[r] = pv[0];
-                s[r + 1] = pv[1];
-            }
-#pragma unroll
-            for (int s2 = 0; s2 < 2; ++s2) {
-                const bf16x8 pf = pack8(pr, s2);
-                const bf16x8 df = pack8(s, s2);
-                const int rb = qb * 32 + s2 * 16 + hi * 4;
-#pragma unroll
-                for (int db = 0; db < 2; ++db) {
-                    av[db] = __builtin_amdgcn_mfma_f32_32x32x16_bf16(frag_tr(tG, db, rb, rb + 8, lane), pf, av[db], 0, 0, 0);
-                    ak[db] = __builtin_amdgcn_mfma_f32_32x32x16_bf16(frag_tr(tQ, db, rb, rb + 8, lane), df, ak[db], 0, 0, 0);
-                }
-            }
-        }
-    }
-    };
-    if constexpr (CAUSAL) tiles(std::integral_constant<int, 2>{}, qt0, nqt);
-    else {
+    const unsigned lds0 = lds_addr_of(smem);
+    if constexpr (CAUSAL) {
+#define ATTN_MODE 2
+#define ATTN_STEADY false
+#define ATTN_QT_BEGIN qt0
+#define ATTN_QT_END nqt
+#include "attention_dkv_tiles.h"
+#undef ATTN_MODE
+#undef ATTN_STEADY
+#undef ATTN_QT_BEGIN
+#undef ATTN_QT_END
+    } else {
         const int nfull = kb0 + 32 * NW - 1 >= p.Lk ? 0 : (p.Lq >> 6);
-        tiles(std::integral_constant<int, 0>{}, 0, nfull);
-        tiles(std::integral_constant<int, 1>{}, nfull, nqt);
+        const int ks = GS ? nfull : max(nfull - 1, 0);
+        if constexpr (GS) {
+#define ATTN_MODE 0
+#define ATTN_STEADY false
+#define ATTN_QT_BEGIN 0
+#define ATTN_QT_END nfull
+#include "attention_dkv_tiles.h"
+#undef ATTN_MODE
+#undef ATTN_STEADY
+#undef ATTN_QT_BEGIN
+#undef ATTN_QT_END
+        } else {
+#define ATTN_MODE 0
+#define ATTN_STEADY true
+#define ATTN_QT_BEGIN 0
+#define ATTN_QT_END ks
+#include "attention_dkv_tiles.h"
+#undef ATTN_MODE
+#undef ATTN_STEADY
+#undef ATTN_QT_BEGIN
+#undef ATTN_QT_END
+        }
+#define ATTN_MODE 1
+#define ATTN_STEADY false
+#define ATTN_QT_BEGIN ks
+#define ATTN_QT_END nqt
+#include "attention_dkv_tiles.h"
+#undef ATTN_MODE
+#undef ATTN_STEADY
+#undef ATTN_QT_BEGIN
+#undef ATTN_QT_END
     }
     bf16* DK = p.dk + (long)b * p.Lk * p.lddk + h * 64;
     bf16* DV = p.dv + (long)b * p.Lk * p.lddv + h * 64;
@@ -778,6 +659,7 @@
 int g_attn_bwd_waves = 4;
 int g_attn_fwd_waves = 4;
 int g_attn_fwd_pipe = 0;
+int g_attn_addressing = 3;
 int g_attn_plain_order = 0;
 int g_attn_defer = DW_ATTN_DEFER;
 int g_attn_ablate = 0;
@@ -812,6 +694,7 @@
     if (causal != 0 && causal != 1 && causal != 2) return DW_EINVAL;
     if (causal == 2 && Lk < Lq) return DW_EINVAL;
     p.coff = causal == 2 ? Lk - Lq : 0;
+    p.half_skip = (g_attn_addressing >> 1) & 1;
     hipStream_t s = (hipStream_t)stream;
     if (Lq == 1 && causal != 1 && g_attn_decode && Lk <= 8192) {
         const size_t smem = (((size_t)Lk + 3) & ~(size_t)3) * 4 + 16 * 64 * 4 + 2 * 16 * 4;
@@ -838,11 +721,13 @@
     }
 #endif
     const int g8 = (Lq + 255) / 256;
+    const bool gs = !(g_attn_addressing & 1) || ldk != ldv;
     if (causal) hipLaunchKernelGGL(attn_fwd_kernel<true>, grid, block, 0, s, p);
     else if (g_attn_fwd_pipe == 2 && Lk > 64) hipLaunchKernelGGL((attn_fwd_pipe_kernel<4, 2>), grid, block, 0, s, p);
     else if (g_attn_fwd_pipe && Lk > 64) hipLaunchKernelGGL((attn_fwd_pipe_kernel<4, 3>), grid, block, 0, s, p);
-    else if (g_attn_fwd_waves == 8 && g8 * 2 == g4 && (long)g8 * H * B >= 512)
+    else if (g_attn_fwd_waves == 8 && !gs && g8 * 2 == g4 && (long)g8 * H * B >= 512)
         hipLaunchKernelGGL((attn_fwd_kernel<false, 8>), dim3(g8 * H * B), dim3(512), 0, s, p);
+    else if (gs) hipLaunchKernelGGL((attn_fwd_kernel<false, 4, 0, false, true>), grid, block, 0, s, p);
     else hipLaunchKernelGGL(attn_fwd_kernel<false>, grid, block, 0, s, p);
     DW_CHECK_LAUNCH();
     return DW_OK;
@@ -869,9 +754,12 @@
     p.q_start = q_start; p.q_len = q_len; p.kv_start = kv_start; p.kv_len = kv_len; p.kv_B = kv_batches;
     p.plain_order = g_attn_plain_order;
     p.defer = (float)g_attn_defer;
+    p.half_skip = (g_attn_addressing >> 1) & 1;
     hipStream_t s = (hipStream_t)stream;
     dim3 grid(((max_q + 127) / 128) * H * n_seq), block(256);
+    const bool gs = !(g_attn_addressing & 1) || ldk != ldv;
     if (causal) hipLaunchKernelGGL((attn_fwd_kernel<true, 4, 0, true>), grid, block, 0, s, p);
+    else if (gs) hipLaunchKernelGGL((attn_fwd_kernel<false, 4, 0, true, true>), grid, block, 0, s, p);
     else hipLaunchKernelGGL((attn_fwd_kernel<false, 4, 0, true>), grid, block, 0, s, p);
     DW_CHECK_LAUNCH();
     return DW_OK;
@@ -918,6 +806,7 @@
     dim3 gq(q4 * H * B), gk(k4 * H * B), block(256);
     p.plain_order = g_attn_plain_order;
     p.defer = (float)g_attn_defer;
+    p.half_skip = (g_attn_addressing >> 1) & 1;
     const int fs = g_attn_bwd_stage;
     if (causal) {
         hipLaunchKernelGGL((attn_bwd_dq_kernel<true, false>), gq, block, 0, s, p);
@@ -927,9 +816,9 @@
         const bool dq12 = g_attn_bwd_waves == 12 && q12 * 3 == q4 && (long)q12 * H * B >= 256;
         const bool dkv12 = g_attn_bwd_waves == 12 && k12 * 3 == k4 && (long)k12 * H * B >= 256;
         if (dq12) hipLaunchKernelGGL((attn_bwd_dq_kernel<false, true, 12>), dim3(q12 * H * B), dim3(768), 0, s, p);
-        else if (fs & 1) hipLaunchKernelGGL((attn_bwd_dq_kernel<false, true>), gq, block, 0, s, p);
-        else hipLaunchKernelGGL((attn_bwd_dq_kernel<false, false>), gq, block, 0, s, p);
-        if (dkv12) hipLaunchKernelGGL((attn_bwd_dkv_kernel<false, false, 3, 12>), dim3(k12 * H * B), dim3(768), 0, s, p);
+        else if ((fs & 1) && ldk == ldv) hipLaunchKernelGGL((attn_bwd_dq_kernel<false, false>), gq, block, 0, s, p);
+        else hipLaunchKernelGGL((attn_bwd_dq_kernel<false, true>), gq, block, 0, s, p);
+        if (dkv12) hipLaunchKernelGGL((attn_bwd_dkv_kernel<false, true, 3, 12>), dim3(k12 * H * B), dim3(768), 0, s, p);
         else if ((fs & 6) == 6) hipLaunchKernelGGL((attn_bwd_dkv_kernel<false, true, 3>), gk, block, 0, s, p);
         else if (fs & 4) hipLaunchKernelGGL((attn_bwd_dkv_kernel<false, false, 3>), gk, block, 0, s, p);
         else if (fs & 2) hipLaunchKernelGGL((attn_bwd_dkv_kernel<false, true, 2>), gk, block, 0, s, p);
diff --git a/distil_whisper_amd/csrc/attention_dkv_tiles.h b/distil_whisper_amd/csrc/attention_dkv_tiles.h
--- /dev/null
+++ b/distil_whisper_amd/csrc/attention_dkv_tiles.h
@@ -0,0 +1,87 @@
+{
+    int lane_o = lane;
+    asm volatile("" : "+v"(lane_o));
+    const int hi_o = lane_o >> 5, key_o = kb0 + wave * 32 + (lane_o & 31);
+    const bool k_ok_o = key_o < p.Lk;
+    unsigned voQ = 0, voG = 0;
+    if constexpr (ATTN_STEADY) {
+        voQ = stage_lane_off(p.ldq, wave, lane_o);
+        voG = stage_lane_off(p.lddo, wave, lane_o);
+    }
+    for (int qt = ATTN_QT_BEGIN; qt < ATTN_QT_END; ++qt) {
+        const int buf = (qt - qt0) & 1;
+        wait_vm0_seen();
+        __syncthreads();
+        if constexpr (ATTN_STEADY) {
+            const unsigned l1 = lds0 + (buf ^ 1) * 17408;
+            stage_full64<NW>(Q + (long)((qt + 1) * 64) * p.ldq, p.ldq, voQ, l1, wave);
+            stage_full64<NW>(DO + (long)((qt + 1) * 64) * p.lddo, p.lddo, voG, l1 + 8192, wave);
+            const unsigned lo = (unsigned)lane_o * 4u;
+            if constexpr (NW == 4) glds4_so(((wave & 1) ? DEL : LSE) + (qt + 1) * 64, lo, l1 + 16384 + wave * 256);
+            else if (wave < 2) glds4_so((wave ? DEL : LSE) + (qt + 1) * 64, lo, l1 + 16384 + wave * 256);
+        } else if (qt + 1 < nqt) {
+            int lane_s = lane_o;
+            asm volatile("" : "+v"(lane_s));
+            stage(qt + 1, buf ^ 1, lane_s);
+        }
+        const char* tQ = smem + buf * 17408;
+        const char* tG = tQ + 8192;
+        const float* tL = (const float*)(tQ + 16384);
+        const float* tD = tL + 64;
+        const bool need_mask = ATTN_MODE == 1 || (ATTN_MODE == 2 && (((qt + 1) * 64 > p.Lq) || (wk0 + 31 >= p.Lk) || (CAUSAL && wk0 + 31 > qt * 64)));
+        if (CAUSAL && wk0 > qt * 64 + 63) continue;
+        if (DW_ATTN_IDLE_SKIP && wk0 >= p.Lk) continue;
+        const bool dead1 = DW_ATTN_HALF_SKIP && need_mask && p.half_skip && qt * 64 + 32 >= p.Lq;
+        const bool dead0 = CAUSAL && DW_ATTN_HALF_SKIP && need_mask && p.half_skip && wk0 > qt * 64 + 31;
+#pragma unroll
+        for (int qb = 0; qb < 2; ++qb) {
+            if (qb == 1 ? dead1 : dead0) continue;
+            f32x16 s, dp;
+#pragma unroll
+            for (int g = 0; g < 4; ++g) {
+                const int ql = qb * 32 + g * 8 + hi * 4;
+                const f32x4 l4 = *(const f32x4*)(tL + ql);
+                const f32x4 d4 = *(const f32x4*)(tD + ql);
+#pragma unroll
+                for (int e = 0; e < 4; ++e) { s[g * 4 + e] = l4[e]; dp[g * 4 + e] = d4[e]; }
+            }
+#pragma unroll
+            for (int kk = 0; kk < 4; ++kk) {
+                s = __builtin_amdgcn_mfma_f32_32x32x16_bf16(frag_rows(tQ, qb, kk, lane), kf[kk], s, 0, 0, 0);
+                dp = __builtin_amdgcn_mfma_f32_32x32x16_bf16(frag_rows(tG, qb, kk, lane), vf[kk], dp, 0, 0, 0);
+            }
+            f32x16 pr;
+            const f32x2 c2 = {c, c};
+#pragma unroll
+            for (int r = 0; r < 16; r += 2) {
+                f32x2 t = {s[r], s[r + 1]};
+                t = t * c2;
+                f32x2 pv = {__builtin_amdgcn_exp2f(t[0]), __builtin_amdgcn_exp2f(t[1])};
+                if (need_mask) {
+#pragma unroll
+                    for (int e = 0; e < 2; ++e) {
+                        const int qi = qt * 64 + qb * 32 + ((r + e) & 3) + 8 * ((r + e) >> 2) + 4 * hi_o;
+                        pv[e] = (qi < p.Lq && k_ok_o && (!CAUSAL || key_o <= qi)) ? pv[e] : 0.f;
+                    }
+                }
+                pr[r] = pv[0];
+                pr[r + 1] = pv[1];
+                const f32x2 d2 = {dp[r], dp[r + 1]};
+                pv = pv * d2;
+                s[r] = pv[0];
+                s[r + 1] = pv[1];
+            }
+#pragma unroll
+            for (int s2 = 0; s2 < 2; ++s2) {
+                const bf16x8 pf = pack8(pr, s2);
+                const bf16x8 df = pack8(s, s2);
+                const int rb = qb * 32 + s2 * 16 + hi * 4;
+#pragma unroll
+                for (int db = 0; db < 2; ++db) {
+                    av[db] = __builtin_amdgcn_mfma_f32_32x32x16_bf16(frag_tr(tG, db, rb, rb + 8, lane), pf, av[db], 0, 0, 0);
+                    ak[db] = __builtin_amdgcn_mfma_f32_32x32x16_bf16(frag_tr(tQ, db, rb, rb + 8, lane), df, ak[db], 0, 0, 0);
+                }
+            }
+        }
+    }
+}
diff --git a/distil_whisper_amd/csrc/attention_dq_tiles.h b/distil_whisper_amd/csrc/attention_dq_tiles.h
--- /dev/null
+++ b/distil_whisper_amd/csrc/attention_dq_tiles.h
@@ -0,0 +1,67 @@
+{
+    int lane_o = lane;
+    asm volatile("" : "+v"(lane_o));
+    const int hi_o = lane_o >> 5, q_o = qb0 + wave * 32 + (lane_o & 31);
+    unsigned voK = 0;
+    if constexpr (ATTN_STEADY) voK = stage_lane_off(p.ldk, wave, lane_o);
+    for (int kt = ATTN_KT_BEGIN; kt < ATTN_KT_END; ++kt) {
+        const int buf = kt & 1;
+        wait_vm0();
+        __syncthreads();
+        if constexpr (ATTN_STEADY) {
+            const unsigned l1 = lds0 + (buf ^ 1) * 16384;
+            stage_full64<NW>(K + (long)((kt + 1) * 64) * p.ldk, p.ldk, voK, l1, wave);
+            stage_full64<NW>(V + (long)((kt + 1) * 64) * p.ldk, p.ldk, voK, l1 + 8192, wave);
+        } else if (kt + 1 < nkt) {
+            int lane_s = lane_o;
+            asm volatile("" : "+v"(lane_s));
+            stage_tile64<NW>(K, p.ldk, (kt + 1) * 64, p.Lk, smem + (buf ^ 1) * 16384, wave, lane_s);
+            stage_tile64<NW>(V, p.ldv, (kt + 1) * 64, p.Lk, smem + (buf ^ 1) * 16384 + 8192, wave, lane_s);
+        }
+        const char* tK = smem + buf * 16384;
+        const char* tV = tK + 8192;
+        const int wq0 = qb0 + wave * 32;
+        const bool need_mask = ATTN_MODE == 1 || (ATTN_MODE == 2 && (((kt + 1) * 64 > p.Lk) || (CAUSAL && kt * 64 + 63 > wq0)));
+        if (CAUSAL && kt * 64 > wq0 + 31) continue;
+        if (DW_ATTN_IDLE_SKIP && wq0 >= p.Lq) continue;
+        const bool dead1 = DW_ATTN_HALF_SKIP && need_mask && p.half_skip && ((kt * 64 + 32 >= p.Lk) || (CAUSAL && kt * 64 + 32 > wq0 + 31));
+#pragma unroll
+        for (int kb = 0; kb < 2; ++kb) {
+            if (kb == 1 && dead1) continue;
+            f32x16 s, dp;
+#pragma unroll
+            for (int r = 0; r < 16; ++r) { s[r] = s0; dp[r] = dp0; }
+#pragma unroll
+            for (int kk = 0; kk < 4; ++kk) {
+                s = __builtin_amdgcn_mfma_f32_32x32x16_bf16(frag_rows(tK, kb, kk, lane), qf[kk], s, 0, 0, 0);
+                dp = __builtin_amdgcn_mfma_f32_32x32x16_bf16(frag_rows(tV, kb, kk, lane), gf[kk], dp, 0, 0, 0);
+            }
+            const f32x2 c2 = {c, c};
+#pragma unroll
+            for (int r = 0; r < 16; r += 2) {
+                f32x2 t = {s[r], s[r + 1]};
+                t = t * c2;
+                f32x2 pv = {__builtin_amdgcn_exp2f(t[0]), __builtin_amdgcn_exp2f(t[1])};
+                if (need_mask) {
+#pragma unroll
+                    for (int e = 0; e < 2; ++e) {
+                        const int key = kt * 64 + kb * 32 + ((r + e) & 3) + 8 * ((r + e) >> 2) + 4 * hi_o;
+                        pv[e] = (key < p.Lk && (!CAUSAL || key <= q_o)) ? pv[e] : 0.f;
+                    }
+                }
+                const f32x2 d2 = {dp[r], dp[r + 1]};
+                pv = pv * d2;
+                s[r] = pv[0];
+                s[r + 1] = pv[1];
+            }
+#pragma unroll
+            for (int s2 = 0; s2 < 2; ++s2) {
+                const bf16x8 df = pack8(s, s2);
+                const int rb = kb * 32 + s2 * 16 + hi * 4;
+#pragma unroll
+                for (int db = 0; db < 2; ++db)
+                    acc[db] = __builtin_amdgcn_mfma_f32_32x32x16_bf16(frag_tr(tK, db, rb, rb + 8, lane), df, acc[db], 0, 0, 0);
+            }
+        }
+    }
+}
diff --git a/distil_whisper_amd/csrc/attention_fwd_tiles.h b/distil_whisper_amd/csrc/attention_fwd_tiles.h
--- /dev/null
+++ b/distil_whisper_amd/csrc/attention_fwd_tiles.h
@@ -0,0 +1,106 @@
+{
+    unsigned voK = 0; (void)voK;
+    if constexpr (ATTN_STEADY) voK = stage_lane_off(p.ldk, wave, lane);
+    for (int kt = ATTN_KT_BEGIN; kt < ATTN_KT_END; ++kt) {
+        const int buf = kt & 1;
+        if (!(ABL & 16) || kt == 0) {
+            wait_vm0_seen();
+            __syncthreads();
+        }
+        if constexpr (ATTN_STEADY) {
+            if (!(ABL & 8)) {
+                const unsigned l1 = lds0 + (buf ^ 1) * 16384;
+                stage_full64<NW>(K + (long)((kt + 1) * 64) * p.ldk, p.ldk, voK, l1, wave);
+                stage_full64<NW>(V + (long)((kt + 1) * 64) * p.ldk, p.ldk, voK, l1 + 8192, wave);
+            }
+        } else if (kt + 1 < nkt && !(ABL & 8)) {
+            stage_tile64<NW>(K, p.ldk, (kt + 1) * 64, Lk, smem + (buf ^ 1) * 16384, wave, lane);
+            stage_tile64<NW>(V, p.ldv, (kt + 1) * 64, Lk, smem + (buf ^ 1) * 16384 + 8192, wave, lane);
+        }
+        const char* tK = smem + buf * 16384;
+        const char* tV = tK + 8192;
+        if (DW_ATTN_IDLE_SKIP && qb0 + wave * 32 >= Lq) continue;
+        const bool dead1 = DW_ATTN_HALF_SKIP && !CAUSAL && !ATTN_STEADY && p.half_skip && kt * 64 + 32 >= Lk;
+        f32x16 s[2];
+#pragma unroll
+        for (int kb = 0; kb < 2; ++kb) {
+            if (kb == 1 && dead1) continue;
+#pragma unroll
+            for (int r = 0; r < 16; ++r) s[kb][r] = (ABL & 32) ? o[kb][r] : 0.f;
+            if (!(ABL & 32)) {
+#pragma unroll
+                for (int kk = 0; kk < 4; ++kk)
+                    s[kb] = __builtin_amdgcn_mfma_f32_32x32x16_bf16((ABL & 2) ? qf[kk ^ kb] : frag_rows(tK, kb, kk, lane), qf[kk], s[kb], 0, 0, 0);
+            }
+        }
+        const int wq0 = qb0 + wave * 32 + (CAUSAL ? p.coff : 0);
+        const bool need_mask = (!ATTN_STEADY && (kt + 1) * 64 > Lk) || (CAUSAL && kt * 64 + 63 > wq0);
+        if (CAUSAL && kt * 64 > wq0 + 31) continue;
+        float mx = NEG_BIG;
+        if (need_mask) {
+#pragma unroll
+            for (int kb = 0; kb < 2; ++kb) {
+                if (kb == 1 && dead1) continue;
+#pragma unroll
+                for (int r = 0; r < 16; ++r) {
+                    const int key = kt * 64 + kb * 32 + (r & 3) + 8 * (r >> 2) + 4 * hi;
+                    const bool ok = key < Lk && (!CAUSAL || key <= q + p.coff);
+                    s[kb][r] = ok ? s[kb][r] : NEG_BIG;
+                }
+            }
+        }
+#pragma unroll
+        for (int kb = 0; kb < 2; ++kb) {
+            if (kb == 1 && dead1) continue;
+#pragma unroll
+            for (int r = 0; r < 16; ++r) mx = fmaxf(mx, s[kb][r]);
+        }
+        mx = xhalf_max(mx);
+        const bool move = __any((mx - m_run) * c > p.defer);
+        const float m_new = move ? fmaxf(m_run, mx) : m_run;
+        const float mc = m_new * c;
+        f32x2 rs2[2] = {{0.f, 0.f}, {0.f, 0.f}};
+        const f32x2 c2 = {c, c}, mc2 = {mc, mc};
+#pragma unroll
+        for (int kb = 0; kb < 2; ++kb) {
+            if (kb == 1 && dead1) continue;
+#pragma unroll
+            for (int r = 0; r < 16; r += 2) {
+                f32x2 t = {s[kb][r], s[kb][r + 1]};
+                t = t * c2 - mc2;
+                f32x2 pv = {__builtin_amdgcn_exp2f(t[0]), __builtin_amdgcn_exp2f(t[1])};
+                if (ABL & 1) pv = t;
+                s[kb][r] = pv[0];
+                s[kb][r + 1] = pv[1];
+                rs2[(r >> 1) & 1] += pv;
+            }
+        }
+        rs2[0] += rs2[1];
+        float rs = rs2[0][0] + rs2[0][1];
+        rs = xhalf_sum(rs);
+        if (move) {
+            const float alpha = __builtin_amdgcn_exp2f((m_run - m_new) * c);
+            l_run *= alpha;
+#pragma unroll
+            for (int r = 0; r < 16; ++r) { o[0][r] *= alpha; o[1][r] *= alpha; }
+        }
+        l_run += rs;
+        m_run = m_new;
+#pragma unroll
+        for (int kb = 0; kb < 2; ++kb) {
+            if (kb == 1 && dead1) continue;
+#pragma unroll
+            for (int s2 = 0; s2 < 2; ++s2) {
+                const bf16x8 pf = pack8(s[kb], s2);
+                const int rb = kb * 32 + s2 * 16 + hi * 4;
+                if (ABL & 64) {
+                    o[kb][s2] += bf2f(pf[0]) + bf2f(pf[2]) + bf2f(pf[4]) + bf2f(pf[6]);
+                    continue;
+                }
+#pragma unroll
+                for (int db = 0; db < 2; ++db)
+                    o[db] = __builtin_amdgcn_mfma_f32_32x32x16_bf16((ABL & 4) ? qf[db * 2 + s2] : frag_tr(tV, db, rb, rb + 8, lane), pf, o[db], 0, 0, 0);
+            }
+        }
+    }
+}
diff --git a/distil_whisper_amd/csrc/common.h b/distil_whisper_amd/csrc/common.h
--- a/distil_whisper_amd/csrc/common.h
+++ b/distil_whisper_amd/csrc/common.h
@@ -181,6 +181,24 @@
     }
 }
 
+__device__ __forceinline__ unsigned stage_lane_off(long row_stride, int wave, int lane) {
+    const int row = wave * 8 + (lane >> 3);
+    unsigned voff = (unsigned)(row * (int)row_stride + (((lane & 7) ^ swz7(row)) << 3)) * 2u;
+    asm volatile("" : "+v"(voff));
+    return voff;
+}
+template <int NW>
+__device__ __forceinline__ void stage_full64(const bf16* tile, long row_stride, unsigned voff, unsigned lds0, int wave) {
+    static_assert(NW == 4 || NW == 8 || NW == 12 || NW == 2, "chunk c = wave + i * NW: rows 8 c + (lane >> 3)");
+    if constexpr (NW <= 8) {
+#pragma unroll
+        for (int i = 0; i < 8 / NW; ++i)
+            glds16_so(tile + (long)(i * NW * 8) * row_stride, voff, lds0 + (wave + i * NW) * 1024);
+    } else {
+        if (wave < 8) glds16_so(tile, voff, lds0 + wave * 1024);
+    }
+}
+
 __device__ __forceinline__ float wave_sum(float v) {
 #pragma unroll
     for (int o = 32; o > 0; o >>= 1) v += __shfl_xor(v, o);
diff --git a/distil_whisper_amd/csrc/gemm.hip b/distil_whisper_amd/csrc/gemm.hip
--- a/distil_whisper_amd/csrc/gemm.hip
+++ b/distil_whisper_amd/csrc/gemm.hip
@@ -22,6 +22,7 @@
 extern int g_attn_ablate;
 extern int g_attn_fwd_waves;
 extern int g_attn_fwd_pipe;
+extern int g_attn_addressing;
 extern int g_attn_plain_order;
 extern int g_attn_defer;
 extern int g_attn_bwd_waves;
@@ -70,6 +71,7 @@
     if (key == 22) { g_gemm_row_tail = value; return DW_OK; }
     if (key == 25) { if (value < 0 || value > 1) return DW_EINVAL; g_gemm_small_m = value; return DW_OK; }
     if (key == 26) { g_attn_fwd_pipe = value; return DW_OK; }
+    if (key == 27) { if (value < 0 || value > 3) return DW_EINVAL; g_attn_addressing = value; return DW_OK; }
     if (key == 18) { g_attn_plain_order = value; return DW_OK; }
     if (key == 23) { if (value < 0 || value > 64) return DW_EINVAL; g_attn_defer = value; return DW_OK; }
     if (key == 16) { g_attn_fwd_waves = value; return DW_OK; }
```

Result: no change. 2811 (median of 6 runs) (+0.9%).
